# SinOncology/BreakID

Hardware: NVIDIA B200
Metric: read_pairs_per_sec_classified_clustered_refined (higher is better)
Workload: dtype u32/i64 integer + f64 (AHC distances)

## Files before the change

breakid_b200/csrc/bkid_api.cuh:

```cuda
#pragma once

#define GRID1(n, t) (unsigned)div_up((long long)(n), (t))

enum CounterSlot {
  CS_G = 0,
  CS_SD_OUT = 16,
  CS_SDF = 20,
  CS_SORT = 28,
  CS_TOTAL = 32,
  CS_HASH_ERR = 40,
  CS_MAXSPAN = 44,
  CS_FATAL = 46,
  CS_ROOTS = 48,
  CS_MISSING = 50,
  CS_DECODE = 52,
  CS_NC = 64,
  CS_XBAD = 65,
  CS_RG_TICKET = 66,
  CS_SORT_HEAP = 67
};

struct Scratch {
  DBuf keys, keys_alt, vals, vals_alt, hist, scan_tmp, a32, b32, c32, d32, e32;
  int ensure(long long n, cudaStream_t st)
  {
    size_t m = (size_t)std::max<long long>(n, 1);
    BK_TRY(keys.ensure(m * 8, 0, st)); BK_TRY(keys_alt.ensure(m * 8, 0, st));
    BK_TRY(vals.ensure(m * 4, 0, st)); BK_TRY(vals_alt.ensure(m * 4, 0, st));
    BK_TRY(hist.ensure(bk::radix_hist_elems(n) * 4, 0, st));
    BK_TRY(scan_tmp.ensure((bk::scan_tmp_elems(std::max<long long>((long long)bk::radix_hist_elems(n), n)) + 8) * 8, 0, st));
    BK_TRY(a32.ensure(m * 4 + 16, 0, st)); BK_TRY(b32.ensure(m * 4 + 16, 0, st)); BK_TRY(c32.ensure(m * 4 + 16, 0, st));
    BK_TRY(d32.ensure(m * 4 + 16, 0, st)); BK_TRY(e32.ensure(m * 4 + 16, 0, st));
    return 0;
  }
  bk::RadixTmp rt() { return bk::RadixTmp{keys_alt.as<uint64_t>(), vals_alt.as<uint32_t>(), hist.as<uint32_t>(), scan_tmp.as<unsigned long long>()}; }
  void release() { for (DBuf *b : {&keys, &keys_alt, &vals, &vals_alt, &hist, &scan_tmp, &a32, &b32, &c32, &d32, &e32}) b->release(); }
};

struct bkid_decoder;
static void decoder_free(bkid_ctx *c);

struct bkid_ctx {
  bkid_decoder *dec = nullptr;
  std::vector<int32_t> ex_iv;
  DBuf ex_tab, ex_lo, ex_len, ex_pre;
  long long n_excluded = 0;
  int device = 0, n_sm = 148;
  cudaStream_t st = nullptr, st2 = nullptr, st3 = nullptr;
  bkid_params prm;
  int nt = 0;
  std::vector<uint32_t> target_len;
  std::vector<std::string> names;
  std::string err;
  DBuf d_cum, d_bucket_rank, d_canon;
  long long n = 0, cap_n = 0;
  bool borrowed = false;
  DBuf flag, mapq, tid, pos, isize, endpos, cls, cand_bits;
  DBuf isize16, span16;
  int form_isize = 0, form_span = 0;
  long long reserve_hint = 0;
  const int16_t *p_isize16 = nullptr; const uint16_t *p_span16 = nullptr;
  long long n_x = 0;
  DBuf x_rec, x_mtid, x_mpos, x_nh;
  const uint16_t *p_flag = nullptr; const uint8_t *p_mapq = nullptr;
  const int32_t *p_tid = nullptr, *p_pos = nullptr, *p_isize = nullptr, *p_endpos = nullptr;
  const uint32_t *p_x_rec = nullptr; const int32_t *p_x_mtid = nullptr, *p_x_mpos = nullptr; const uint64_t *p_x_nh = nullptr;
  long long n_sa = 0, n_cig = 0, sa_bytes = 0, oc_bytes = 0;
  DBuf sa_rec, cig_off, cig_ops, sa_off, sa_txt, oc_off, oc_txt;
  DBuf seq_off, seq4, seq_len; long long seq_bytes = 0; bool have_seq = false;
  const uint32_t *p_seq_off = nullptr; const uint8_t *p_seq4 = nullptr; const int32_t *p_seq_len = nullptr;
  const uint32_t *p_sa_rec = nullptr, *p_cig_off = nullptr, *p_cig_ops = nullptr, *p_sa_off = nullptr, *p_oc_off = nullptr;
  const uint8_t *p_sa_txt = nullptr, *p_oc_txt = nullptr;
  std::vector<DBuf> nib;
  std::vector<uint64_t> nib_len;
  DBuf d_nib_ptr, d_nib_len;
  bool classified = false, have_stats = false, scanned = false, clustered = false, refined = false;
  double mean = 0, sd = 0;
  long long sum_abs = 0, cnt_insert = 0, sd_total = 0;
  unsigned long long sum_sq = 0, xmax = 0;
  long long n_cand_k1 = 0;
  int sd_kub = 0;
  bool sd_fast_pending = false;
  DBuf tile_cand, counters, cand_idx, cand, bucket_rank_of;
  long long n_cand = 0;
  DBuf pairs0, pairs_tmp, bucket_off0;
  long long np0 = 0; int nb = 0;
  DBuf X, Y, bucket_of_pair;
  DBuf cur1, curb1, seg1;
  long long n1 = 0;
  DBuf mem_pair, mem_bucket, mem_cluster;
  long long n2 = 0;
  std::vector<int32_t> roots_per_bucket;
  DBuf sdtab, sdlut; bool sd_prepared = false; double sd_mean = 0;
  DBuf clusters, clusters_out, sarows, work, cov, depth, evoff, valid, name_key, name_row;
  const void *rows_ptr = nullptr; long long n_rows = 0, n_evcap = 0; int maxspan = 1; bool clusters_ranked = false;
  long long n_clusters = 0, n_called = 0;
  Scratch sc;
  DBuf tmpA, tmpB, tmpC, tmpD, tmpE, tmpF, tmpG, tmpH;
  DBuf dist_send, dist_recv, dist_rows;
  DBuf sortheap;
  DBuf sortbig;
  DBuf dist_scalars;
  bkid_timings tm;
  cudaEvent_t ev[16];
  cudaEvent_t ev_run[2];
  cudaEvent_t ev_side[2];
  cudaEvent_t ev_w[4];
  bool k8_attr_set = false;
  bool sd_side_pending = false;
  bool maxspan_cached = false, maxspan_pending = false;
  long long launches0 = 0;
};

struct SubTimer {
  cudaStream_t st; bool on; std::vector<std::pair<std::string, cudaEvent_t>> ev;
  explicit SubTimer(cudaStream_t s) : st(s), on(getenv("BKID_DEBUG_TIMING") != nullptr) { mark("start"); }
  void mark(const char *name) { if (!on) return; cudaEvent_t e; cudaEventCreate(&e); cudaEventRecord(e, st); ev.push_back({name, e}); }
  ~SubTimer() {
    if (!on) return;
    cudaStreamSynchronize(st);
    for (size_t i = 1; i < ev.size(); ++i) { float ms = 0; cudaEventElapsedTime(&ms, ev[i - 1].second, ev[i].second); fprintf(stderr, "[bkid-timing] %-28s %8.3f ms\n", ev[i].first.c_str(), ms); }
    for (auto &e : ev) cudaEventDestroy(e.second);
  }
};

static int fail(bkid_ctx *c, int code, const std::string &msg)
{
  if (c) c->err = msg;
  else g_create_err = msg;
  return code;
}
#define CU(c, x) do { cudaError_t e__ = (x); if (e__ != cudaSuccess) { bk_set_cuda_error(e__, __FILE__, __LINE__); return fail((c), e__ == cudaErrorMemoryAllocation ? BKID_ERR_NOMEM : BKID_ERR_CUDA, g_last_cuda_err); } } while (0)
#define TRY(c, x) do { int rc__ = (x); if (rc__ != 0) { if ((c)->err.empty()) (c)->err = g_last_cuda_err; return rc__; } } while (0)

static int sync_check(bkid_ctx *c)
{
  CU(c, cudaStreamSynchronize(c->st));
  CU(c, cudaGetLastError());
  return 0;
}

static int exact_sort_segments(bkid_ctx *c, uint32_t *key, uint32_t *val, const uint32_t *seg_off, int nseg, long long n)
{
  if (n < 2 || nseg <= 0) return 0;
  cudaStream_t st = c->st;
  size_t seg_bytes = ((size_t)n / 2 + 16) * sizeof(Seg);
  TRY(c, c->tmpA.ensure(seg_bytes, 0, st));
  TRY(c, c->tmpB.ensure(seg_bytes, 0, st));
  TRY(c, c->tmpC.ensure(seg_bytes, 0, st));
  TRY(c, c->tmpD.ensure((size_t)n * 4 + 16, 0, st));
  TRY(c, c->tmpE.ensure((size_t)n * 4 + 16, 0, st));
  TRY(c, c->counters.ensure(256, 0, st));
  unsigned *cnt = c->counters.as<unsigned>() + CS_SORT;
  CU(c, cudaMemsetAsync(cnt, 0, 16, st));
  Seg *act[2] = {c->tmpA.as<Seg>(), c->tmpB.as<Seg>()};
  Seg *term = c->tmpC.as<Seg>();
  TRY(c, c->tmpH.ensure(seg_bytes, 0, st));
  Seg *small = c->tmpH.as<Seg>();
  TRY(c, c->sortheap.ensure(((size_t)n / IS_SMALL + 16) * sizeof(Seg), 0, st));
  Seg *heapl = c->sortheap.as<Seg>();
  unsigned *n_heap = c->counters.as<unsigned>() + CS_SORT_HEAP;
  CU(c, cudaMemsetAsync(n_heap, 0, 4, st));
  const bool big_possible = n > (long long)IS_BIG;
  const size_t maxbig = (size_t)(n / IS_BIG) + 2, maxtiles = (size_t)(n / IS_BTILE) + maxbig + 2;
  BigSeg *big[2] = {nullptr, nullptr};
  unsigned long long *bigcnt = nullptr, *status = nullptr;
  unsigned *tickets = nullptr;
  if (big_possible) {
    TRY(c, c->sortbig.ensure(64 + 2 * maxbig * sizeof(BigSeg) + maxtiles * 8, 0, st));
    char *base = (char *)c->sortbig.p;
    bigcnt = (unsigned long long *)base; tickets = (unsigned *)(base + 16);
    big[0] = (BigSeg *)(base + 64); big[1] = big[0] + maxbig;
    status = (unsigned long long *)(big[1] + maxbig);
    CU(c, cudaMemsetAsync(base, 0, 64, st));
    CU(c, cudaMemsetAsync(status, 0, maxtiles * 8, st));
  }
  BK_LAUNCH(is_init_roots, GRID1(nseg, 256), 256, 0, st, seg_off, nseg, act[0], cnt + 0, small, cnt + 3, term, cnt + 2, big[0], bigcnt);
  int lg = 0;
  for (long long t = n; t > 1; t >>= 1) ++lg;
  int max_levels = 2 * lg + 2;
  int cur = 0;
  bool any_big = big_possible;
  for (int level = 0; level < max_levels; ++level) {
    if (level > 0 && (level % 4) == 0) {
      unsigned h = 0;
      unsigned long long hb = 0;
      CU(c, cudaMemcpyAsync(&h, cnt + cur, 4, cudaMemcpyDeviceToHost, st));
      if (any_big) CU(c, cudaMemcpyAsync(&hb, bigcnt + cur, 8, cudaMemcpyDeviceToHost, st));
      CU(c, cudaStreamSynchronize(st));
      if (hb == 0) any_big = false;
      if (h == 0 && !any_big) break;
    }
    CU(c, cudaMemsetAsync(cnt + (cur ^ 1), 0, 4, st));
    if (any_big) {
      BK_LAUNCH(is_big_part, 592, IS_THREADS, 0, st, key, val, big[cur], bigcnt + cur, tickets, status, c->tmpD.as<uint32_t>(), c->tmpE.as<uint32_t>(),
                bigcnt + (cur ^ 1), tickets + 1, heapl, n_heap);
      BK_LAUNCH(is_big_swap, 592, IS_THREADS, 0, st, key, val, big[cur], bigcnt + cur, tickets + 1, c->tmpD.as<uint32_t>(), c->tmpE.as<uint32_t>(),
                act[cur ^ 1], cnt + (cur ^ 1), small, cnt + 3, term, cnt + 2, big[cur ^ 1], bigcnt + (cur ^ 1), tickets, status);
    }
    BK_LAUNCH(is_level, 592, IS_THREADS, 0, st, key, val, act[cur], cnt + cur, act[cur ^ 1], cnt + (cur ^ 1), small, cnt + 3, term, cnt + 2,
              c->tmpD.as<uint32_t>(), c->tmpE.as<uint32_t>(), heapl, n_heap);
    cur ^= 1;
  }
  BK_LAUNCH(is_heap, 148, 256, IS_HEAP_SMEM_ELEMS * 8 + 16, st, key, val, heapl, n_heap);
  BK_LAUNCH(is_small, 2368, ISS_WARPS * 32, 0, st, key, val, small, cnt + 3);
  BK_LAUNCH(is_terminal, 592, 128, 0, st, key, val, term, cnt + 2);
  return 0;
}

static int sort_current_by(bkid_ctx *c, uint32_t *cur, long long n, const uint32_t *coord, const uint32_t *seg_off, int nseg)
{
  if (n < 2) return 0;
  TRY(c, c->tmpF.ensure((size_t)n * 4 + 16, 0, c->st));
  uint32_t *key = c->tmpF.as<uint32_t>();
  BK_LAUNCH(gather_u32, GRID1(n, 256), 256, 0, c->st, coord, cur, n, key);
  return exact_sort_segments(c, key, cur, seg_off, nseg, n);
}

static int mask_pass(bkid_ctx *c, const uint32_t *cur, const uint32_t *curb, const uint32_t *seg, long long n, int nseg, const uint32_t *X, const uint32_t *Y,
                     long long distance, uint32_t *cur_out, uint32_t *curb_out, uint32_t *seg_out, long long *n_out)
{
  cudaStream_t st = c->st;
  if (n == 0) { CU(c, cudaMemsetAsync(seg_out, 0, (size_t)(nseg + 1) * 4, st)); *n_out = 0; return 0; }
  TRY(c, c->sc.ensure(n, st));
  uint32_t *cnt = c->sc.a32.as<uint32_t>(), *off = c->sc.b32.as<uint32_t>();
  unsigned long long *tot = (unsigned long long *)(c->counters.as<unsigned>() + CS_TOTAL);
  BK_LAUNCH(k4_mask_count, GRID1(n, 256), 256, 0, st, cur, curb, seg, n, X, Y, distance, cnt);
  bk::exclusive_scan<uint32_t, uint32_t>(cnt, off, n, c->sc.scan_tmp.as<unsigned long long>(), tot, st);
  unsigned long long h = 0;
  CU(c, cudaMemcpyAsync(&h, tot, 8, cudaMemcpyDeviceToHost, st));
  CU(c, cudaStreamSynchronize(st));
  BK_LAUNCH(k4_mask_write, GRID1(n, 256), 256, 0, st, cur, curb, n, cnt, off, cur_out, curb_out);
  BK_LAUNCH(k4_new_offsets, GRID1(nseg + 1, 256), 256, 0, st, seg, nseg, off, n, h, seg_out);
  *n_out = (long long)h;
  return 0;
// ... 200 lines not shown
    unsigned *rg_ticket = c->counters.as<unsigned>() + CS_RG_TICKET;
    CU(c, cudaMemsetAsync(rg_ticket, 0, 4, st));
    BK_LAUNCH(ahc_rg_ties, 148 * 4, 128, 0, st, v, g, curb, bucket_flag, RG_LO, bucket_events, head_pos, tot, rg_ticket);
    BK_LAUNCH(ahc_rg_write, GRID1(n, 256), 256, 0, st, v, g, curb, n, bucket_flag, RG_LO);
  }
  T_.mark("ahc: replay rank form (global)");
  BK_LAUNCH(ahc_bucket_exact, (unsigned)nseg, 32, 0, st, v, bucket_comp_off, (uint32_t)nseg, bucket_flag, 4096u);
  T_.mark("ahc: replay+exact");
  unsigned *cnt = c->counters.as<unsigned>() + CS_ROOTS;
  CU(c, cudaMemsetAsync(cnt, 0, 4, st));
  uint64_t *rkey = c->sc.keys.as<uint64_t>();
  uint32_t *rnode = c->sc.vals.as<uint32_t>();
  BK_LAUNCH(ahc_final_roots, GRID1(ncomp, 128), 128, 0, st, v, ncomp, rkey, rnode, cnt, merges_pb);
  unsigned nroot = 0;
  CU(c, cudaMemcpyAsync(&nroot, cnt, 4, cudaMemcpyDeviceToHost, st)); CU(c, cudaStreamSynchronize(st));
  std::vector<unsigned> merges(nseg);
  std::vector<uint32_t> segh(nseg + 1);
  CU(c, cudaMemcpyAsync(merges.data(), merges_pb, (size_t)nseg * 4, cudaMemcpyDeviceToHost, st));
  CU(c, cudaMemcpyAsync(segh.data(), seg, (size_t)(nseg + 1) * 4, cudaMemcpyDeviceToHost, st));
  CU(c, cudaStreamSynchronize(st));
  for (int b = 0; b < nseg; ++b) c->roots_per_bucket[b] = (int32_t)(segh[b + 1] - segh[b]) - (int32_t)merges[b];
  if (nroot == 0) return sync_check(c);
  bk::radix_sort_pairs(rkey, rnode, nroot, 0, 32 + bbits, c->sc.rt(), st);
  uint32_t *rsize = c->sc.a32.as<uint32_t>(), *roff = c->sc.b32.as<uint32_t>(), *rhead = c->sc.e32.as<uint32_t>();
  BK_LAUNCH(ahc_root_sizes, GRID1(nroot, 128), 128, 0, st, v, rkey, rnode, nroot, rsize, rhead);
  BK_LAUNCH(ahc_root_firsts, GRID1(nroot, 128), 128, 0, st, rhead, nroot, rkey, bucket_first_root);
  bk::exclusive_scan<uint32_t, uint32_t>(rsize, roff, nroot, stmp, tot, st);
  unsigned long long nm = 0;
  CU(c, cudaMemcpyAsync(&nm, tot, 8, cudaMemcpyDeviceToHost, st)); CU(c, cudaStreamSynchronize(st));
  size_t mb = (size_t)std::max<unsigned long long>(nm, 1) * 4 + 16;
  TRY(c, c->mem_pair.ensure(mb, 0, st)); TRY(c, c->mem_bucket.ensure(mb, 0, st)); TRY(c, c->mem_cluster.ensure(mb, 0, st));
  TRY(c, c->tmpE.ensure(mb, 0, st));
  BK_LAUNCH(ahc_emit, GRID1(nroot, 4), 128, 0, st, v, rkey, rnode, roff, bucket_first_root, nroot, c->tmpE.as<uint32_t>(), c->mem_cluster.as<int32_t>(), c->mem_bucket.as<uint32_t>());
  BK_LAUNCH(gather_u32, GRID1(nm, 256), 256, 0, st, cur, c->tmpE.as<uint32_t>(), (long long)nm, c->mem_pair.as<uint32_t>());
  c->n2 = (long long)nm;
  T_.mark("ahc: final roots+emit");
  return sync_check(c);
}

__global__ void fast_member_keys(const uint32_t *__restrict__ curb, const int32_t *__restrict__ cl, long long n, uint64_t *__restrict__ key, uint32_t *__restrict__ val)
{
  long long p = (long long)blockIdx.x * blockDim.x + threadIdx.x;
  if (p < n) { key[p] = ((uint64_t)curb[p] << 32) | (uint32_t)cl[p]; val[p] = (uint32_t)p; }
}
__global__ void fast_member_write(const uint64_t *__restrict__ key, const uint32_t *__restrict__ val, const uint32_t *__restrict__ cur, long long n,
                                  uint32_t *__restrict__ mem_pair, uint32_t *__restrict__ mem_bucket, int32_t *__restrict__ mem_cluster)
{
  long long p = (long long)blockIdx.x * blockDim.x + threadIdx.x;
  if (p < n) { mem_pair[p] = cur[val[p]]; mem_bucket[p] = (uint32_t)(key[p] >> 32); mem_cluster[p] = (int32_t)(key[p] & 0xffffffffu); }
}

static int cluster_fast(bkid_ctx *c, const uint32_t *cur, const uint32_t *curb, const uint32_t *seg, long long n, int nseg, const uint32_t *X, const uint32_t *Y, double w,
                        long long np0)
{
  cudaStream_t st = c->st;
  c->n2 = 0;
  c->roots_per_bucket.assign(nseg, 0);
  if (n == 0) return 0;
  int min_reads = c->prm.min_reads;
  TRY(c, c->sc.ensure(std::max(n, np0) + 8, st));
  size_t m = (size_t)n * 4 + 64, sb = (size_t)(nseg + 2) * 4;
  TRY(c, c->tmpG.ensure(4 * m + 4 * sb + (size_t)np0 * 8 + 64, 0, st));
  uint32_t *curA = c->tmpG.as<uint32_t>(), *curbA = curA + n + 8, *curB = curbA + n + 8, *curbB = curB + n + 8;
  uint32_t *segA = curbB + n + 8, *segB = segA + nseg + 2;
  uint32_t *k1 = segB + nseg + 2, *k2 = k1 + np0;
  uint32_t *keep = c->sc.a32.as<uint32_t>(), *off = c->sc.b32.as<uint32_t>();
  long long na = 0, nb2 = 0, nc = 0;
  BK_LAUNCH(fast_sweep, GRID1(nseg, 64), 64, 0, st, cur, seg, (uint32_t)nseg, X, w, min_reads, k1, keep);
  TRY(c, compact_pass(c, cur, curb, seg, n, nseg, keep, curA, curbA, segA, off, &na));
  TRY(c, sort_current_by(c, curA, na, Y, segA, nseg));
  if (na > 0) BK_LAUNCH(fast_sweep, GRID1(nseg, 64), 64, 0, st, curA, segA, (uint32_t)nseg, Y, w, min_reads, k2, keep);
  TRY(c, compact_pass(c, curA, curbA, segA, na, nseg, keep, curB, curbB, segB, off, &nb2));
  TRY(c, sort_current_by(c, curB, nb2, X, segB, nseg));
  if (nb2 == 0) return sync_check(c);
  int32_t *cl = (int32_t *)c->sc.c32.as<uint32_t>();
  int32_t *ncl = (int32_t *)c->sc.d32.as<uint32_t>();
  BK_LAUNCH(fast_number, GRID1(nseg, 64), 64, 0, st, curB, segB, (uint32_t)nseg, k1, k2, min_reads, cl, keep, ncl);
  CU(c, cudaMemcpyAsync(c->roots_per_bucket.data(), ncl, (size_t)nseg * 4, cudaMemcpyDeviceToHost, st));
  uint32_t *curC = curA, *curbC = curbA;
  bk::exclusive_scan<uint32_t, uint32_t>(keep, off, nb2, c->sc.scan_tmp.as<unsigned long long>(), (unsigned long long *)(c->counters.as<unsigned>() + CS_TOTAL), st);
  unsigned long long h = 0;
  CU(c, cudaMemcpyAsync(&h, c->counters.as<unsigned>() + CS_TOTAL, 8, cudaMemcpyDeviceToHost, st)); CU(c, cudaStreamSynchronize(st));
  nc = (long long)h;
  if (nc == 0) return 0;
  BK_LAUNCH(compact_write, GRID1(nb2, 256), 256, 0, st, curB, curbB, keep, off, nb2, curC, curbC);
  uint32_t *clC = c->sc.e32.as<uint32_t>();
  BK_LAUNCH(compact_write, GRID1(nb2, 256), 256, 0, st, (const uint32_t *)cl, curbB, keep, off, nb2, clC, c->sc.vals_alt.as<uint32_t>() );
  uint64_t *key = c->sc.keys.as<uint64_t>();
  uint32_t *val = c->sc.vals.as<uint32_t>();
  BK_LAUNCH(fast_member_keys, GRID1(nc, 256), 256, 0, st, curbC, (const int32_t *)clC, nc, key, val);
  int bbits = 1; while ((1ll << bbits) < nseg + 1) ++bbits;
  bk::radix_sort_pairs(key, val, nc, 0, 32 + bbits, c->sc.rt(), st);
  size_t mb = (size_t)nc * 4 + 16;
  TRY(c, c->mem_pair.ensure(mb, 0, st)); TRY(c, c->mem_bucket.ensure(mb, 0, st)); TRY(c, c->mem_cluster.ensure(mb, 0, st));
  BK_LAUNCH(fast_member_write, GRID1(nc, 256), 256, 0, st, key, val, curC, nc, c->mem_pair.as<uint32_t>(), c->mem_bucket.as<uint32_t>(), c->mem_cluster.as<int32_t>());
  c->n2 = nc;
  return sync_check(c);
}

extern "C" {

int bkid_abi_version(void) { return BKID_ABI_VERSION; }

const char *bkid_last_error(const bkid_ctx *ctx) { return ctx ? ctx->err.c_str() : g_create_err.c_str(); }

void bkid_default_params(bkid_params *p)
{
  p->qual = 20; p->times = 2; p->fast = 0; p->min_reads = 2; p->bp_pos_error = 2; p->mismatch_num = 10; p->sd_mult = 3; p->validate_align = 0;
}

bkid_ctx *bkid_create(int device, const bkid_header *hdr, const bkid_params *params)
{
  int ndev = 0;
  cudaError_t e = cudaGetDeviceCount(&ndev);
  if (e != cudaSuccess || ndev == 0) { g_create_err = std::string("no usable CUDA device (there is no CPU fallback): ") + cudaGetErrorString(e); return nullptr; }
  if (device < 0 || device >= ndev) { g_create_err = "device index out of range"; return nullptr; }
  if (!hdr || hdr->n_targets < 0) { g_create_err = "bad header"; return nullptr; }
  if (cudaSetDevice(device) != cudaSuccess) { g_create_err = "cudaSetDevice failed"; return nullptr; }
  bkid_ctx *c = new bkid_ctx();
  c->device = device;
  cudaDeviceGetAttribute(&c->n_sm, cudaDevAttrMultiProcessorCount, device);
  if (params) c->prm = *params; else bkid_default_params(&c->prm);
  if (cudaStreamCreateWithFlags(&c->st, cudaStreamNonBlocking) != cudaSuccess) { g_create_err = "cudaStreamCreate failed"; delete c; return nullptr; }
  cudaStreamCreateWithFlags(&c->st2, cudaStreamNonBlocking);
  cudaStreamCreateWithFlags(&c->st3, cudaStreamNonBlocking);
  for (auto &ev : c->ev) cudaEventCreate(&ev);
  for (auto &ev : c->ev_run) cudaEventCreate(&ev);
  for (auto &ev : c->ev_side) cudaEventCreate(&ev);
  for (auto &ev : c->ev_w) cudaEventCreateWithFlags(&ev, cudaEventDisableTiming);
  c->nt = hdr->n_targets;
  for (int i = 0; i < c->nt; ++i) { c->target_len.push_back(hdr->target_len[i]); c->names.emplace_back(hdr->target_name[i]); }
  int nt = c->nt, m = nt + 1;
  std::vector<uint32_t> cum(nt + 1, 0);
  for (int i = 0; i < nt; ++i) cum[i + 1] = cum[i] + c->target_len[i];
  std::vector<std::pair<std::string, int>> bn;
  for (int a = 0; a < m; ++a)
    for (int b = 0; b < m; ++b) bn.push_back({(a ? c->names[a - 1] : std::string("*")) + "_" + (b ? c->names[b - 1] : std::string("*")), a * m + b});
  std::sort(bn.begin(), bn.end());
  std::vector<int32_t> rank((size_t)m * m);
  for (size_t r = 0; r < bn.size(); ++r) rank[bn[r].second] = (int32_t)r;
  std::vector<uint64_t> canon(nt ? nt : 1);
  for (int i = 0; i < nt; ++i) canon[i] = chr_code((const uint8_t *)c->names[i].data(), (uint32_t)c->names[i].size());
  bool ok = c->d_cum.ensure((size_t)(nt + 1) * 4, 0, c->st) == 0 && c->d_bucket_rank.ensure(rank.size() * 4, 0, c->st) == 0 &&
            c->d_canon.ensure(canon.size() * 8, 0, c->st) == 0 && c->counters.ensure(1024, 0, c->st) == 0 &&
            c->d_nib_ptr.ensure((size_t)(nt + 1) * 8, 0, c->st) == 0 && c->d_nib_len.ensure((size_t)(nt + 1) * 8, 0, c->st) == 0;
  if (!ok) { g_create_err = "device allocation failed: " + g_last_cuda_err; delete c; return nullptr; }
  cudaMemcpy(c->d_cum.p, cum.data(), (size_t)(nt + 1) * 4, cudaMemcpyHostToDevice);
  cudaMemcpy(c->d_bucket_rank.p, rank.data(), rank.size() * 4, cudaMemcpyHostToDevice);
  cudaMemcpy(c->d_canon.p, canon.data(), canon.size() * 8, cudaMemcpyHostToDevice);
  cudaMemset(c->d_nib_ptr.p, 0, (size_t)(nt + 1) * 8);
  cudaMemset(c->d_nib_len.p, 0, (size_t)(nt + 1) * 8);
  c->nib.resize(nt); c->nib_len.assign(nt, 0);
  cudaFuncSetAttribute(sd_resolve, cudaFuncAttributeMaxDynamicSharedMemorySize, SD_BLOCK * 9);
  cudaFuncSetAttribute(is_heap, cudaFuncAttributeMaxDynamicSharedMemorySize, (int)(IS_HEAP_SMEM_ELEMS * 8 + 16));
  cudaFuncSetAttribute(ahc_replay_smem, cudaFuncAttributeMaxDynamicSharedMemorySize, 49 * 4096);
  cudaFuncSetAttribute(ahc_replay_rank, cudaFuncAttributeMaxDynamicSharedMemorySize, 49 * 4096);
  memset(&c->tm, 0, sizeof c->tm);
  if (cudaGetLastError() != cudaSuccess) { g_create_err = "CUDA error during create"; delete c; return nullptr; }
  return c;
}

void bkid_destroy(bkid_ctx *c)
{
  if (!c) return;
  cudaSetDevice(c->device);
  cudaStreamSynchronize(c->st);
  decoder_free(c);
  for (DBuf *b : {&c->d_cum, &c->d_bucket_rank, &c->d_canon, &c->flag, &c->mapq, &c->tid, &c->pos, &c->isize, &c->endpos, &c->isize16, &c->span16, &c->cand_bits, &c->x_rec, &c->x_mtid, &c->x_mpos, &c->x_nh, &c->cls,
                  &c->sa_rec, &c->cig_off, &c->cig_ops, &c->sa_off, &c->sa_txt, &c->oc_off, &c->oc_txt, &c->seq_off, &c->seq4, &c->seq_len, &c->d_nib_ptr, &c->d_nib_len, &c->tile_cand, &c->counters,
                  &c->cand_idx, &c->cand, &c->bucket_rank_of, &c->pairs0, &c->pairs_tmp, &c->bucket_off0, &c->X, &c->Y, &c->bucket_of_pair, &c->cur1, &c->curb1, &c->seg1, &c->mem_pair,
                  &c->mem_bucket, &c->mem_cluster, &c->sdtab, &c->sdlut, &c->clusters, &c->clusters_out, &c->sarows, &c->name_key, &c->name_row, &c->ex_tab, &c->ex_lo, &c->ex_len, &c->ex_pre, &c->work, &c->cov, &c->depth, &c->evoff, &c->valid, &c->tmpA, &c->tmpB, &c->tmpC, &c->tmpD, &c->tmpE, &c->tmpF, &c->tmpG, &c->tmpH, &c->dist_send, &c->dist_recv, &c->dist_rows, &c->dist_scalars, &c->sortbig, &c->sortheap})
    b->release();
  for (auto &b : c->nib) b.release();
  c->sc.release();
  for (auto &ev : c->ev) cudaEventDestroy(ev);
  for (auto &ev : c->ev_run) cudaEventDestroy(ev);
  for (auto &ev : c->ev_side) cudaEventDestroy(ev);
  for (auto &ev : c->ev_w) cudaEventDestroy(ev);
  cudaStreamDestroy(c->st2);
  cudaStreamDestroy(c->st3);
  cudaStreamDestroy(c->st);
  delete c;
}

static void invalidate(bkid_ctx *c)
{
  if (c->sd_side_pending || c->sd_fast_pending) { cudaStreamSynchronize(c->st2); c->sd_side_pending = false; c->sd_fast_pending = false; }
  if (c->maxspan_pending) { cudaStreamSynchronize(c->st3); c->maxspan_pending = false; }
  c->classified = c->have_stats = c->scanned = c->clustered = c->refined = false; c->sd_prepared = false; c->maxspan_cached = false;
}

static int reserve_impl(bkid_ctx *c, long long n, long long n_x, long long n_sa, long long n_cig, long long sa_b, long long oc_b)
{
  cudaStream_t st = c->st;
  if (c->borrowed) return fail(c, BKID_ERR_ARG, "context holds borrowed device columns; bkid_reset first");
  size_t k = (size_t)c->n;
  TRY(c, c->flag.ensure((size_t)n * 2 + 64, k * 2, st)); TRY(c, c->mapq.ensure((size_t)n + 64, k, st));
  TRY(c, c->tid.ensure((size_t)n * 4 + 64, k * 4, st)); TRY(c, c->pos.ensure((size_t)n * 4 + 64, k * 4, st));
  if (c->form_isize == 1) TRY(c, c->isize.ensure((size_t)n * 4 + 64, k * 4, st));
  if (c->form_isize == 2) TRY(c, c->isize16.ensure((size_t)n * 2 + 64, k * 2, st));
  if (c->form_span == 1) TRY(c, c->endpos.ensure((size_t)n * 4 + 64, k * 4, st));
  if (c->form_span == 2) TRY(c, c->span16.ensure((size_t)n * 2 + 64, k * 2, st));
  size_t kx = (size_t)c->n_x;
  TRY(c, c->x_rec.ensure((size_t)n_x * 4 + 64, kx * 4, st)); TRY(c, c->x_mtid.ensure((size_t)n_x * 4 + 64, kx * 4, st));
  TRY(c, c->x_mpos.ensure((size_t)n_x * 4 + 64, kx * 4, st)); TRY(c, c->x_nh.ensure((size_t)n_x * 16 + 64, kx * 16, st));
  size_t s = (size_t)c->n_sa;
  TRY(c, c->sa_rec.ensure((size_t)n_sa * 4 + 64, s * 4, st));
  TRY(c, c->cig_off.ensure((size_t)(n_sa + 1) * 4 + 64, (s + 1) * 4, st));
  TRY(c, c->sa_off.ensure((size_t)(n_sa + 1) * 4 + 64, (s + 1) * 4, st));
  TRY(c, c->oc_off.ensure((size_t)(n_sa + 1) * 4 + 64, (s + 1) * 4, st));
  TRY(c, c->cig_ops.ensure((size_t)n_cig * 4 + 64, (size_t)c->n_cig * 4, st));
  TRY(c, c->sa_txt.ensure((size_t)sa_b + 64, (size_t)c->sa_bytes, st));
  TRY(c, c->oc_txt.ensure((size_t)oc_b + 64, (size_t)c->oc_bytes, st));
  return 0;
}

int bkid_reserve(bkid_ctx *c, int64_t n, int64_t n_x, int64_t n_sa, int64_t n_cig, int64_t sa_b, int64_t oc_b)
{
  if (!c) return BKID_ERR_ARG;
  cudaSetDevice(c->device);
  c->reserve_hint = std::max<long long>(c->reserve_hint, n);
  return reserve_impl(c, std::max<long long>(n, c->n), std::max<long long>(n_x, c->n_x), std::max<long long>(n_sa, c->n_sa), std::max<long long>(n_cig, c->n_cig),
                      std::max<long long>(sa_b, c->sa_bytes), std::max<long long>(oc_b, c->oc_bytes));
}

__global__ void add_offset_u32(uint32_t *p, long long n, uint32_t d)
{
  long long i = (long long)blockIdx.x * blockDim.x + threadIdx.x;
  if (i < n) p[i] += d;
}

__global__ void widen_isize16(const int16_t *__restrict__ src, long long n, int32_t *__restrict__ dst)
{
  long long i = (long long)blockIdx.x * blockDim.x + threadIdx.x;
  if (i < n) dst[i] = (int32_t)src[i];
}
__global__ void widen_span16(const int32_t *__restrict__ pos, const uint16_t *__restrict__ span, long long n, int32_t *__restrict__ endpos)
{
  long long i = (long long)blockIdx.x * blockDim.x + threadIdx.x;
  if (i < n) endpos[i] = pos[i] + (int32_t)span[i];
}
__global__ void widen_tid_runs(const uint32_t *__restrict__ start, const int32_t *__restrict__ rtid, int nruns, long long n, int32_t *__restrict__ tid)
{
  long long i = (long long)blockIdx.x * blockDim.x + threadIdx.x;
  if (i >= n) return;
  int a = 0, b = nruns;
  while (b - a > 1) { int m = (a + b) >> 1; if ((long long)start[m] <= i) a = m; else b = m; }
  tid[i] = rtid[a];
}

static void set_ptrs(bkid_ctx *c)
{
  c->p_flag = c->flag.as<uint16_t>(); c->p_mapq = c->mapq.as<uint8_t>(); c->p_tid = c->tid.as<int32_t>(); c->p_pos = c->pos.as<int32_t>();
  c->p_isize = c->form_isize == 2 ? nullptr : c->isize.as<int32_t>(); c->p_isize16 = c->form_isize == 2 ? c->isize16.as<int16_t>() : nullptr;
  c->p_endpos = c->form_span == 2 ? nullptr : c->endpos.as<int32_t>(); c->p_span16 = c->form_span == 2 ? c->span16.as<uint16_t>() : nullptr;
  c->p_x_rec = c->x_rec.as<uint32_t>(); c->p_x_mtid = c->x_mtid.as<int32_t>(); c->p_x_mpos = c->x_mpos.as<int32_t>(); c->p_x_nh = c->x_nh.as<uint64_t>();
  c->p_sa_rec = c->sa_rec.as<uint32_t>(); c->p_cig_off = c->cig_off.as<uint32_t>(); c->p_cig_ops = c->cig_ops.as<uint32_t>();
  c->p_seq_off = c->seq_off.as<uint32_t>(); c->p_seq4 = c->seq4.as<uint8_t>(); c->p_seq_len = c->seq_len.as<int32_t>();
  c->p_sa_off = c->sa_off.as<uint32_t>(); c->p_sa_txt = c->sa_txt.as<uint8_t>(); c->p_oc_off = c->oc_off.as<uint32_t>(); c->p_oc_txt = c->oc_txt.as<uint8_t>();
}

static int settle_forms(bkid_ctx *c, int want_isize, int want_span, long long n_new)
{
  cudaStream_t st = c->st;
  long long n0 = c->n;
  size_t cap = (size_t)std::max<long long>(n0 + n_new, c->reserve_hint);
  if (c->form_isize == 0) c->form_isize = want_isize;
  else if (c->form_isize == 2 && want_isize == 1) {
    TRY(c, c->isize.ensure(cap * 4 + 64, 0, st));
    if (n0) BK_LAUNCH(widen_isize16, GRID1(n0, 256), 256, 0, st, c->isize16.as<int16_t>(), n0, c->isize.as<int32_t>());
    c->form_isize = 1;
  }
  if (c->form_span == 0) c->form_span = want_span;
  else if (c->form_span == 2 && want_span == 1) {
    TRY(c, c->endpos.ensure(cap * 4 + 64, 0, st));
    if (n0) BK_LAUNCH(widen_span16, GRID1(n0, 256), 256, 0, st, c->pos.as<int32_t>(), c->span16.as<uint16_t>(), n0, c->endpos.as<int32_t>());
    c->form_span = 1;
  }
  return 0;
}

static int push_impl(bkid_ctx *c, const bkid_batch *b, cudaMemcpyKind kind)
{
  if (!c || !b || b->n < 0 || b->n_sa < 0 || b->n_x < 0) return c ? fail(c, BKID_ERR_ARG, "bad batch") : BKID_ERR_ARG;
  if (b->n > 0 && ((!b->isize && !b->isize16) || (!b->endpos && !b->span16) || (!b->tid && (b->n_tid_runs <= 0 || !b->tid_run_start || !b->tid_run_tid))))
    return fail(c, BKID_ERR_ARG, "bad batch: a dense column is missing in both its wide and its narrow form");
  cudaSetDevice(c->device);
  cudaStream_t st = c->st;
  if ((unsigned long long)(c->n + b->n) >= 0xffffffffull) return fail(c, BKID_ERR_ARG, "more than 2^32-1 records per context");
  invalidate(c);
  cudaEventRecord(c->ev[0], st);
  long long n0 = c->n, s0 = c->n_sa, x0 = c->n_x;
  uint32_t ncig = 0, nsa_b = 0, noc_b = 0;
  if (b->n_sa > 0) {
    if (kind == cudaMemcpyHostToDevice) { ncig = b->cig_off[b->n_sa]; nsa_b = b->sa_off[b->n_sa]; noc_b = b->oc_off[b->n_sa]; }
    else {
      CU(c, cudaMemcpy(&ncig, b->cig_off + b->n_sa, 4, cudaMemcpyDeviceToHost));
      CU(c, cudaMemcpy(&nsa_b, b->sa_off + b->n_sa, 4, cudaMemcpyDeviceToHost));
      CU(c, cudaMemcpy(&noc_b, b->oc_off + b->n_sa, 4, cudaMemcpyDeviceToHost));
    }
  }
  if (b->n > 0) TRY(c, settle_forms(c, b->isize ? 1 : 2, b->endpos ? 1 : 2, b->n));
  TRY(c, reserve_impl(c, std::max<long long>(n0 + b->n, c->reserve_hint), x0 + b->n_x, s0 + b->n_sa, c->n_cig + ncig, c->sa_bytes + nsa_b, c->oc_bytes + noc_b));
  size_t n = (size_t)b->n;
  if (n) {
    cudaStream_t sw = c->st3;
    const bool widen_i = b->isize16 && !b->isize && c->form_isize == 1, widen_s = b->span16 && !b->endpos && c->form_span == 1;
    size_t stage = (widen_i ? n * 2 : 0) + (widen_s ? n * 2 : 0) + (b->tid ? 0 : (size_t)b->n_tid_runs * 8) + 64;
    TRY(c, c->tmpH.ensure(stage, 0, st));
    char *sp = (char *)c->tmpH.p;
    bool widened = false;
    if (b->tid) CU(c, cudaMemcpyAsync(c->tid.as<int32_t>() + n0, b->tid, n * 4, kind, st));
    else {
      uint32_t *rs = (uint32_t *)sp; sp += (size_t)b->n_tid_runs * 4;
      int32_t *rt = (int32_t *)sp; sp += (size_t)b->n_tid_runs * 4;
      CU(c, cudaMemcpyAsync(rs, b->tid_run_start, (size_t)b->n_tid_runs * 4, kind, st));
      CU(c, cudaMemcpyAsync(rt, b->tid_run_tid, (size_t)b->n_tid_runs * 4, kind, st));
      CU(c, cudaEventRecord(c->ev_w[0], st)); CU(c, cudaStreamWaitEvent(sw, c->ev_w[0], 0));
      BK_LAUNCH(widen_tid_runs, GRID1(n, 256), 256, 0, sw, rs, rt, (int)b->n_tid_runs, (long long)n, c->tid.as<int32_t>() + n0);
      widened = true;
    }
    if (c->form_isize == 2) CU(c, cudaMemcpyAsync(c->isize16.as<int16_t>() + n0, b->isize16, n * 2, kind, st));
    else if (b->isize) CU(c, cudaMemcpyAsync(c->isize.as<int32_t>() + n0, b->isize, n * 4, kind, st));
    else {
      int16_t *s16 = (int16_t *)sp; sp += n * 2;
      CU(c, cudaMemcpyAsync(s16, b->isize16, n * 2, kind, st));
      CU(c, cudaEventRecord(c->ev_w[1], st)); CU(c, cudaStreamWaitEvent(sw, c->ev_w[1], 0));
      BK_LAUNCH(widen_isize16, GRID1(n, 256), 256, 0, sw, s16, (long long)n, c->isize.as<int32_t>() + n0);
      widened = true;
    }
    CU(c, cudaMemcpyAsync(c->pos.as<int32_t>() + n0, b->pos, n * 4, kind, st));
    if (c->form_span == 2) CU(c, cudaMemcpyAsync(c->span16.as<uint16_t>() + n0, b->span16, n * 2, kind, st));
    else if (b->endpos) CU(c, cudaMemcpyAsync(c->endpos.as<int32_t>() + n0, b->endpos, n * 4, kind, st));
    else {
      uint16_t *e16 = (uint16_t *)sp; sp += n * 2;
      CU(c, cudaMemcpyAsync(e16, b->span16, n * 2, kind, st));
      CU(c, cudaEventRecord(c->ev_w[2], st)); CU(c, cudaStreamWaitEvent(sw, c->ev_w[2], 0));
      BK_LAUNCH(widen_span16, GRID1(n, 256), 256, 0, sw, c->pos.as<int32_t>() + n0, e16, (long long)n, c->endpos.as<int32_t>() + n0);
      widened = true;
    }
    CU(c, cudaMemcpyAsync(c->flag.as<uint16_t>() + n0, b->flag, n * 2, kind, st));
    CU(c, cudaMemcpyAsync(c->mapq.as<uint8_t>() + n0, b->mapq, n, kind, st));
    if (widened) { CU(c, cudaEventRecord(c->ev_w[3], sw)); CU(c, cudaStreamWaitEvent(st, c->ev_w[3], 0)); }
  }
  size_t nx = (size_t)b->n_x;
  if (nx) {
    CU(c, cudaMemcpyAsync(c->x_rec.as<uint32_t>() + x0, b->x_rec, nx * 4, kind, st));
    CU(c, cudaMemcpyAsync(c->x_mtid.as<int32_t>() + x0, b->x_mtid, nx * 4, kind, st));
    CU(c, cudaMemcpyAsync(c->x_mpos.as<int32_t>() + x0, b->x_mpos, nx * 4, kind, st));
    CU(c, cudaMemcpyAsync(c->x_nh.as<uint64_t>() + 2 * x0, b->x_name_hash, nx * 16, kind, st));
    if (n0) BK_LAUNCH(add_offset_u32, GRID1(nx, 256), 256, 0, st, c->x_rec.as<uint32_t>() + x0, (long long)nx, (uint32_t)n0);
  }
  size_t ns = (size_t)b->n_sa;
  if (ns) {
    CU(c, cudaMemcpyAsync(c->sa_rec.as<uint32_t>() + s0, b->sa_rec, ns * 4, kind, st));
    CU(c, cudaMemcpyAsync(c->cig_off.as<uint32_t>() + s0, b->cig_off, (ns + 1) * 4, kind, st));
    CU(c, cudaMemcpyAsync(c->sa_off.as<uint32_t>() + s0, b->sa_off, (ns + 1) * 4, kind, st));
    CU(c, cudaMemcpyAsync(c->oc_off.as<uint32_t>() + s0, b->oc_off, (ns + 1) * 4, kind, st));
    if (ncig) CU(c, cudaMemcpyAsync(c->cig_ops.as<uint32_t>() + c->n_cig, b->cig_ops, (size_t)ncig * 4, kind, st));
    if (nsa_b) CU(c, cudaMemcpyAsync(c->sa_txt.as<uint8_t>() + c->sa_bytes, b->sa_txt, nsa_b, kind, st));
    if (noc_b) CU(c, cudaMemcpyAsync(c->oc_txt.as<uint8_t>() + c->oc_bytes, b->oc_txt, noc_b, kind, st));
    if (n0) BK_LAUNCH(add_offset_u32, GRID1(ns, 256), 256, 0, st, c->sa_rec.as<uint32_t>() + s0, (long long)ns, (uint32_t)n0);
    if (c->n_cig) BK_LAUNCH(add_offset_u32, GRID1(ns + 1, 256), 256, 0, st, c->cig_off.as<uint32_t>() + s0, (long long)ns + 1, (uint32_t)c->n_cig);
    if (c->sa_bytes) BK_LAUNCH(add_offset_u32, GRID1(ns + 1, 256), 256, 0, st, c->sa_off.as<uint32_t>() + s0, (long long)ns + 1, (uint32_t)c->sa_bytes);
    if (c->oc_bytes) BK_LAUNCH(add_offset_u32, GRID1(ns + 1, 256), 256, 0, st, c->oc_off.as<uint32_t>() + s0, (long long)ns + 1, (uint32_t)c->oc_bytes);
  } else if (s0 == 0) {
    CU(c, cudaMemsetAsync(c->cig_off.p, 0, 4, st)); CU(c, cudaMemsetAsync(c->sa_off.p, 0, 4, st)); CU(c, cudaMemsetAsync(c->oc_off.p, 0, 4, st));
  }
  if (ns) {
    if (b->seq_off && b->seq4 && b->seq_len && (s0 == 0 || c->have_seq)) {
      uint32_t nseq_b = 0;
      if (kind == cudaMemcpyHostToDevice) nseq_b = b->seq_off[ns];
      else CU(c, cudaMemcpy(&nseq_b, b->seq_off + ns, 4, cudaMemcpyDeviceToHost));
      TRY(c, c->seq_off.ensure((size_t)(s0 + ns + 1) * 4 + 64, (size_t)(s0 + 1) * 4, st));
      TRY(c, c->seq_len.ensure((size_t)(s0 + ns) * 4 + 64, (size_t)s0 * 4, st));
      TRY(c, c->seq4.ensure((size_t)c->seq_bytes + nseq_b + 64, (size_t)c->seq_bytes, st));
      CU(c, cudaMemcpyAsync(c->seq_off.as<uint32_t>() + s0, b->seq_off, (ns + 1) * 4, kind, st));
      CU(c, cudaMemcpyAsync(c->seq_len.as<int32_t>() + s0, b->seq_len, ns * 4, kind, st));
      if (nseq_b) CU(c, cudaMemcpyAsync(c->seq4.as<uint8_t>() + c->seq_bytes, b->seq4, nseq_b, kind, st));
      if (c->seq_bytes) BK_LAUNCH(add_offset_u32, GRID1(ns + 1, 256), 256, 0, st, c->seq_off.as<uint32_t>() + s0, (long long)ns + 1, (uint32_t)c->seq_bytes);
      c->seq_bytes += nseq_b; c->have_seq = true;
    } else c->have_seq = false;
  }
  c->n += b->n; c->n_x += b->n_x; c->n_sa += b->n_sa; c->n_cig += ncig; c->sa_bytes += nsa_b; c->oc_bytes += noc_b;
  set_ptrs(c);
  cudaEventRecord(c->ev[1], st);
  TRY(c, sync_check(c));
  float ms = 0; cudaEventElapsedTime(&ms, c->ev[0], c->ev[1]);
  c->tm.h2d += ms;
  return 0;
}

int bkid_push_batch(bkid_ctx *c, const bkid_batch *b) { return push_impl(c, b, cudaMemcpyHostToDevice); }

int bkid_push_batch_device(bkid_ctx *c, const bkid_batch *b)
{
  if (!c || !b) return BKID_ERR_ARG;
  if (c->n == 0 && !c->borrowed && c->flag.p == nullptr) {
    cudaSetDevice(c->device);
    if ((unsigned long long)b->n >= 0xffffffffull) return fail(c, BKID_ERR_ARG, "more than 2^32-1 records per context");
    if (b->n > 0 && (!b->tid || (!b->isize && !b->isize16) || (!b->endpos && !b->span16)))
      return fail(c, BKID_ERR_ARG, "bkid_push_batch_device needs tid and the insert-size / span columns (wide or narrow) resident on the device");
    invalidate(c);
    c->borrowed = true;
    c->n = b->n; c->n_sa = b->n_sa; c->n_x = b->n_x;
    c->p_flag = b->flag; c->p_mapq = b->mapq; c->p_tid = b->tid; c->p_pos = b->pos;
    c->p_isize = b->isize; c->p_isize16 = b->isize ? nullptr : b->isize16;
    c->p_endpos = b->endpos; c->p_span16 = b->endpos ? nullptr : b->span16;
    c->form_isize = b->isize ? 1 : 2; c->form_span = b->endpos ? 1 : 2;
    c->p_x_rec = b->x_rec; c->p_x_mtid = b->x_mtid; c->p_x_mpos = b->x_mpos; c->p_x_nh = b->x_name_hash;
    c->p_sa_rec = b->sa_rec; c->p_cig_off = b->cig_off; c->p_cig_ops = b->cig_ops; c->p_sa_off = b->sa_off; c->p_sa_txt = b->sa_txt;
    c->p_oc_off = b->oc_off; c->p_oc_txt = b->oc_txt;
    c->p_seq_off = b->seq_off; c->p_seq4 = b->seq4; c->p_seq_len = b->seq_len; c->have_seq = b->seq_off && b->seq4 && b->seq_len;
    return 0;
  }
  return push_impl(c, b, cudaMemcpyDeviceToDevice);
}

int bkid_reset(bkid_ctx *c)
{
  if (!c) return BKID_ERR_ARG;
  cudaSetDevice(c->device);
  cudaStreamSynchronize(c->st);
  invalidate(c);
  c->n = c->n_x = c->n_sa = c->n_cig = c->sa_bytes = c->oc_bytes = 0;
  c->seq_bytes = 0; c->have_seq = false;
  c->borrowed = false;
  c->form_isize = c->form_span = 0;
  set_ptrs(c);
  memset(&c->tm, 0, sizeof c->tm);
  c->launches0 = g_bk_launches;
  return 0;
}

int bkid_set_exclude(bkid_ctx *c, int64_t n_iv, const int32_t *tid, const int32_t *beg, const int32_t *end)
{
  if (!c || n_iv < 0 || (n_iv > 0 && (!tid || !beg || !end))) return c ? fail(c, BKID_ERR_ARG, "bad exclude intervals") : BKID_ERR_ARG;
  cudaSetDevice(c->device);
  std::vector<std::array<int32_t, 3>> v;
  for (int64_t k = 0; k < n_iv; ++k) {
    if (tid[k] < 0 || tid[k] >= c->nt) return fail(c, BKID_ERR_ARG, "exclude interval on an unknown target");
    int32_t b = beg[k] < 0 ? 0 : beg[k];
    if (end[k] > b) v.push_back({tid[k], b, end[k]});
  }
  std::sort(v.begin(), v.end());
  c->ex_iv.clear();
  for (auto &x : v) {
    size_t m = c->ex_iv.size();
    if (m && c->ex_iv[m - 3] == x[0] && x[1] <= c->ex_iv[m - 1]) { if (x[2] > c->ex_iv[m - 1]) c->ex_iv[m - 1] = x[2]; }
    else { c->ex_iv.push_back(x[0]); c->ex_iv.push_back(x[1]); c->ex_iv.push_back(x[2]); }
  }
  invalidate(c);
  return 0;
}

static ISizeCol isize_col(const bkid_ctx *c) { return ISizeCol{c->p_isize, c->p_isize16}; }

static int classify_impl(bkid_ctx *c)
{
  if (c->classified) return 0;
  cudaStream_t st = c->st;
  long long n = c->n;
  int ntiles = div_up(std::max<long long>(n, 1), K1_TILE);
  TRY(c, c->cls.ensure((size_t)n + 64, 0, st));
  TRY(c, c->cand_bits.ensure((size_t)n / 8 + 64, 0, st));
  unsigned long long *g = (unsigned long long *)(c->counters.as<unsigned>() + CS_G);
  CU(c, cudaMemsetAsync(g, 0, 64, st));
  cudaEventRecord(c->ev[2], st);
  const bool i16 = c->p_isize16 != nullptr, s16 = c->p_span16 != nullptr;
  if (n > 0) {
    uint8_t *cls = c->cls.as<uint8_t>();
    int occ = 0;
    if (i16 && s16) cudaOccupancyMaxActiveBlocksPerMultiprocessor(&occ, k1_classify<true, true>, K1_THREADS, 0);
    else if (i16) cudaOccupancyMaxActiveBlocksPerMultiprocessor(&occ, k1_classify<true, false>, K1_THREADS, 0);
    else if (s16) cudaOccupancyMaxActiveBlocksPerMultiprocessor(&occ, k1_classify<false, true>, K1_THREADS, 0);
    else cudaOccupancyMaxActiveBlocksPerMultiprocessor(&occ, k1_classify<false, false>, K1_THREADS, 0);
    ntiles = std::min(ntiles, c->n_sm * std::max(occ, 1));
    if (i16 && s16) BK_LAUNCH((k1_classify<true, true>), (unsigned)ntiles, K1_THREADS, 0, st, c->p_flag, c->p_mapq, c->p_isize, c->p_isize16, c->p_span16, n, c->prm.qual, cls, c->cand_bits.as<uint8_t>(), g);
    else if (i16) BK_LAUNCH((k1_classify<true, false>), (unsigned)ntiles, K1_THREADS, 0, st, c->p_flag, c->p_mapq, c->p_isize, c->p_isize16, c->p_span16, n, c->prm.qual, cls, c->cand_bits.as<uint8_t>(), g);
    else if (s16) BK_LAUNCH((k1_classify<false, true>), (unsigned)ntiles, K1_THREADS, 0, st, c->p_flag, c->p_mapq, c->p_isize, c->p_isize16, c->p_span16, n, c->prm.qual, cls, c->cand_bits.as<uint8_t>(), g);
    else BK_LAUNCH((k1_classify<false, false>), (unsigned)ntiles, K1_THREADS, 0, st, c->p_flag, c->p_mapq, c->p_isize, c->p_isize16, c->p_span16, n, c->prm.qual, cls, c->cand_bits.as<uint8_t>(), g);
  }
  cudaEventRecord(c->ev[3], st);
  int n_iv = (int)(c->ex_iv.size() / 3);
  c->n_excluded = 0;
  unsigned long long ne = 0;
  if (n_iv > 0 && n > 0) {
    TRY(c, c->ex_tab.ensure((size_t)n_iv * 12 + 64, 0, st)); TRY(c, c->ex_lo.ensure((size_t)n_iv * 4 + 64, 0, st));
    TRY(c, c->ex_len.ensure((size_t)n_iv * 4 + 64, 0, st)); TRY(c, c->ex_pre.ensure((size_t)(n_iv + 1) * 8 + 64, 0, st));
    CU(c, cudaMemcpyAsync(c->ex_tab.p, c->ex_iv.data(), (size_t)n_iv * 12, cudaMemcpyHostToDevice, st));
    BK_LAUNCH(ex_ranges, GRID1(n_iv, 128), 128, 0, st, c->p_tid, c->p_pos, n, c->ex_tab.as<int32_t>(), n_iv, c->ex_lo.as<uint32_t>(), c->ex_len.as<uint32_t>());
    BK_LAUNCH(ex_prefix, 1, 32, 0, st, c->ex_len.as<uint32_t>(), n_iv, c->ex_pre.as<unsigned long long>());
    BK_LAUNCH(ex_apply, 148 * 8, 256, 0, st, c->ex_lo.as<uint32_t>(), c->ex_pre.as<unsigned long long>(), n_iv, isize_col(c), c->cls.as<uint8_t>(), c->cand_bits.as<uint8_t>(), g);
    CU(c, cudaMemcpyAsync(&ne, c->ex_pre.as<unsigned long long>() + n_iv, 8, cudaMemcpyDeviceToHost, st));
  }
  unsigned long long h[6] = {0, 0, 0, 0, 0, 0};
  CU(c, cudaMemcpyAsync(h, g, 48, cudaMemcpyDeviceToHost, st));
  TRY(c, sync_check(c));
  c->n_excluded = (long long)ne;
  float ms = 0; cudaEventElapsedTime(&ms, c->ev[2], c->ev[3]);
  c->tm.classify = ms;
  c->sum_abs = (long long)h[G_SUM]; c->cnt_insert = (long long)h[G_CNT]; c->sum_sq = h[G_SQ]; c->n_cand_k1 = (long long)h[G_CAND]; c->xmax = h[G_XMAX];
  if (s16) { c->maxspan = (int)h[G_SPAN] + 1; c->maxspan_cached = true; }
  c->classified = true;
  c->tm.n_records = n;
  return 0;
}

static int sd_upper_binade(unsigned long long sum_abs, unsigned long long cnt, unsigned long long sum_sq, unsigned long long xmax)
{
  if (cnt == 0) return 0;
  if (xmax > 65535ull) return 51;
  unsigned __int128 V = (unsigned __int128)sum_sq * cnt - (unsigned __int128)sum_abs * sum_abs;
  unsigned __int128 T = V / cnt + 1;
  T += (T >> 30) + 2 * (unsigned __int128)cnt + 1024;
  if (T >> 51) return 51;
  int k = 0;
  while ((T >> (k + 1)) != 0) ++k;
  return k;
}

static int sd_prepare_impl(bkid_ctx *c, double mean, cudaStream_t st = nullptr)
{
  if (!st) st = c->st;
  long long n = c->n;
  c->sd_prepared = false;
  if (n <= 0 || c->cnt_insert <= 0) return 0;
  int nb = div_up(std::max<long long>(n, 1), SD_BLOCK);
  TRY(c, c->sdtab.ensure((size_t)nb * (8 + SD_K * 4 + 4 + 8) + 256, 0, st));
  TRY(c, c->sdlut.ensure((size_t)SD_LUT * 8, 0, st));
  char *bp = (char *)c->sdtab.p;
  long long *blkF = (long long *)bp; bp += (size_t)nb * 8;
  double *blkA = (double *)bp; bp += (size_t)nb * 8;
  uint32_t *blkCum = (uint32_t *)bp; bp += (size_t)nb * SD_K * 4;
  uint32_t *blkN = (uint32_t *)bp;
  BK_LAUNCH(sd_build_lut, SD_LUT / 256, 256, 0, st, mean, c->sdlut.as<unsigned long long>());
  BK_LAUNCH(sd_block_stats, (unsigned)nb, SD_THREADS, 0, st, c->cls.as<uint8_t>(), isize_col(c), n, mean, c->sdlut.as<unsigned long long>(), blkF, blkCum, blkN, blkA);
  c->sd_prepared = true; c->sd_mean = mean;
  return 0;
}

static int sd_partial_impl(bkid_ctx *c, double mean, long long t_in, long long *t_out)
{
  cudaStream_t st = c->st;
  long long n = c->n;
  *t_out = t_in;
  if (n <= 0 || c->cnt_insert <= 0) return 0;
  SubTimer T_(st);
  if (!c->sd_prepared || c->sd_mean != mean) TRY(c, sd_prepare_impl(c, mean));
  T_.mark("sd: block stats");
  int nb = div_up(std::max<long long>(n, 1), SD_BLOCK);
  char *bp = (char *)c->sdtab.p;
  long long *blkF = (long long *)bp; bp += (size_t)nb * 8;
  double *blkA = (double *)bp; bp += (size_t)nb * 8;
  uint32_t *blkCum = (uint32_t *)bp; bp += (size_t)nb * SD_K * 4;
  uint32_t *blkN = (uint32_t *)bp;
  long long *out = (long long *)(c->counters.as<unsigned>() + CS_SD_OUT);
  BK_LAUNCH(sd_resolve, 1, SDR_T, SD_BLOCK * 9, st, c->cls.as<uint8_t>(), isize_col(c), n, mean, nb, blkF, blkCum, blkN, blkA, t_in, out);
  T_.mark("sd: resolve");
  long long h[2] = {0, 0};
  CU(c, cudaMemcpyAsync(h, out, 16, cudaMemcpyDeviceToHost, st));
  TRY(c, sync_check(c));
  if (h[1]) {
    BK_LAUNCH(sd_sequential, 1, 1, 0, st, c->cls.as<uint8_t>(), isize_col(c), n, mean, t_in, out);
    CU(c, cudaMemcpyAsync(h, out, 16, cudaMemcpyDeviceToHost, st));
    TRY(c, sync_check(c));
  }
  *t_out = h[0];
  return 0;
}

static int sd_fast_launch(bkid_ctx *c, double mean, int kub, cudaStream_t st)
{
  long long n = c->n;
  unsigned long long *out = (unsigned long long *)(c->counters.as<unsigned>() + CS_SDF);
  CU(c, cudaMemsetAsync(out, 0, 24, st));
  c->sd_kub = kub;
  if (n <= 0 || c->cnt_insert <= 0) return 0;
  double thr = 1.0 - ldexp(1.0, kub - 53);
  int occ = 0;
  if (c->p_isize16) cudaOccupancyMaxActiveBlocksPerMultiprocessor(&occ, sd_fast<true>, 256, 0);
  else cudaOccupancyMaxActiveBlocksPerMultiprocessor(&occ, sd_fast<false>, 256, 0);
  const int grid = c->n_sm * std::max(occ, 1);
  if (c->p_isize16) BK_LAUNCH((sd_fast<true>), grid, 256, 0, st, c->cls.as<uint8_t>(), c->p_isize, c->p_isize16, n, mean, thr, out);
  else BK_LAUNCH((sd_fast<false>), grid, 256, 0, st, c->cls.as<uint8_t>(), c->p_isize, c->p_isize16, n, mean, thr, out);
  return 0;
}
static int sd_fast_collect(bkid_ctx *c, cudaStream_t st, unsigned long long *F, unsigned long long *E)
{
  unsigned long long h[3] = {0, 0, 0};
  CU(c, cudaMemcpyAsync(h, c->counters.as<unsigned>() + CS_SDF, 24, cudaMemcpyDeviceToHost, st));
  CU(c, cudaStreamSynchronize(st));
  CU(c, cudaGetLastError());
  *F = h[0]; *E = h[2] ? ~0ull : h[1];
  if (c->sd_kub >= 51 && c->cnt_insert > 0) *E = ~0ull;
  return 0;
}

static int side_launch(bkid_ctx *c)
{
  cudaStream_t s2 = c->st2;
  long long n = c->n;
  c->mean = (double)c->sum_abs / (double)c->cnt_insert;
  cudaEventRecord(c->ev_side[0], s2);
  TRY(c, sd_fast_launch(c, c->mean, sd_upper_binade((unsigned long long)c->sum_abs, (unsigned long long)c->cnt_insert, c->sum_sq, c->xmax), s2));
  cudaEventRecord(c->ev_side[1], s2);
  c->sd_fast_pending = true;
  if (!c->maxspan_cached) {
    int *mx = (int *)(c->counters.as<unsigned>() + CS_MAXSPAN);
    CU(c, cudaMemsetAsync(mx, 0, 4, c->st3));
    if (n > 0) BK_LAUNCH(max_span_kernel, 1184, 256, 0, c->st3, c->p_pos, c->p_endpos, n, mx);
    c->maxspan_pending = true;
  }
  return 0;
}

static int side_collect(bkid_ctx *c)
{
  unsigned long long F = 0, E = 0;
  TRY(c, sd_fast_collect(c, c->st2, &F, &E));
  c->sd_fast_pending = false;
  float ms = 0; cudaEventElapsedTime(&ms, c->ev_side[0], c->ev_side[1]);
  long long total = (long long)F;
  if (E != 0 && c->n > 0 && c->cnt_insert > 0) {
    cudaEventRecord(c->ev[4], c->st);
    TRY(c, sd_partial_impl(c, c->mean, 0, &total));
    cudaEventRecord(c->ev[5], c->st);
    TRY(c, sync_check(c));
    float ms2 = 0; cudaEventElapsedTime(&ms2, c->ev[4], c->ev[5]);
    ms += ms2;
  }
  c->tm.insert_stats = ms;
  c->sd_total = total;
  c->sd = sqrt((double)c->sd_total / (double)c->cnt_insert);
  c->have_stats = true;
  return 0;
}

static int maxspan_collect(bkid_ctx *c)
{
  if (!c->maxspan_pending) return 0;
  int maxspan = 0;
  CU(c, cudaMemcpyAsync(&maxspan, c->counters.as<unsigned>() + CS_MAXSPAN, 4, cudaMemcpyDeviceToHost, c->st3));
  CU(c, cudaStreamSynchronize(c->st3));
  CU(c, cudaGetLastError());
  c->maxspan = maxspan + 1; c->maxspan_cached = true; c->maxspan_pending = false;
  return 0;
}

int bkid_insert_stats(bkid_ctx *c, double *mean, double *sd)
{
  if (!c) return BKID_ERR_ARG;
  cudaSetDevice(c->device);
  c->err.clear();
  TRY(c, classify_impl(c));
  if (!c->have_stats) {
    cudaStream_t st = c->st;
    c->mean = (double)c->sum_abs / (double)c->cnt_insert;
    cudaEventRecord(c->ev[4], st);
    unsigned long long F = 0, E = 0;
    const bool general_only = getenv("BKID_SD_GENERAL") != nullptr;
    if (!general_only) {
      TRY(c, sd_fast_launch(c, c->mean, sd_upper_binade((unsigned long long)c->sum_abs, (unsigned long long)c->cnt_insert, c->sum_sq, c->xmax), st));
      TRY(c, sd_fast_collect(c, st, &F, &E));
    }
    long long t = (long long)F;
    if ((general_only || E != 0) && c->n > 0 && c->cnt_insert > 0) TRY(c, sd_partial_impl(c, c->mean, 0, &t));
    cudaEventRecord(c->ev[5], st);
    TRY(c, sync_check(c));
    float ms = 0; cudaEventElapsedTime(&ms, c->ev[4], c->ev[5]);
    c->tm.insert_stats = ms;
    c->sd_total = t;
    c->sd = sqrt((double)c->sd_total / (double)c->cnt_insert);
    c->have_stats = true;
  }
  if (mean) *mean = c->mean;
  if (sd) *sd = c->sd;
  return 0;
}

static int extract_candidates(bkid_ctx *c, unsigned long long index_offset, bool with_keys)
{
  TRY(c, classify_impl(c));
  cudaStream_t st = c->st;
  long long n = c->n, nx = c->n_x;
  long long cap = std::min<long long>(c->n_cand_k1, nx);
  c->n_cand = cap;
  unsigned *cs = c->counters.as<unsigned>();
  CU(c, cudaMemsetAsync(cs + CS_NC, 0, 8, st));
  TRY(c, c->cand.ensure((size_t)(cap + 1) * sizeof(bkid_cand), 0, st));
  if (nx <= 0 || n <= 0) return 0;
  int ntiles = div_up(nx, KX_TILE);
  TRY(c, c->sc.ensure(std::max<long long>(cap, ntiles) + 8, st));
  TRY(c, c->tile_cand.ensure((size_t)(ntiles + 1) * 4 * 2 + (size_t)ntiles * KX_THREADS + 64, 0, st));
  uint32_t *tile_cnt = c->tile_cand.as<uint32_t>(), *tile_off = tile_cnt + ntiles + 1;
  uint8_t *is_cand = (uint8_t *)(tile_off + ntiles + 1);
  unsigned long long *tot = (unsigned long long *)(cs + CS_TOTAL);
  BK_LAUNCH(kx_count, (unsigned)ntiles, KX_THREADS, 0, st, c->p_x_rec, nx, c->cand_bits.as<uint8_t>(), n, tile_cnt, is_cand, (int *)(cs + CS_XBAD));
  bk::exclusive_scan<uint32_t, uint32_t>(tile_cnt, tile_off, ntiles, c->sc.scan_tmp.as<unsigned long long>(), tot, st);
  CU(c, cudaMemcpyAsync(cs + CS_NC, tot, 4, cudaMemcpyDeviceToDevice, st));
  if (cap > 0)
    BK_LAUNCH(kx_write, (unsigned)ntiles, KX_THREADS, 0, st, c->p_x_rec, nx, is_cand, n, tile_off, c->p_flag, c->p_mapq, c->p_tid, c->p_pos, c->p_x_mtid, c->p_x_mpos, c->p_x_nh,
              index_offset, c->cand.as<bkid_cand>(), with_keys ? c->sc.keys.as<uint64_t>() : (uint64_t *)nullptr, c->sc.vals.as<uint32_t>());
  return 0;
}
static int check_candidates(bkid_ctx *c, const unsigned *h_nc_bad)
{
  if (h_nc_bad[1]) return fail(c, BKID_ERR_ARG, "the sparse mate/name table is not strictly ascending or points outside the batch (x_rec)");
  if ((long long)h_nc_bad[0] != c->n_cand_k1)
    return fail(c, BKID_ERR_ARG, "a discordant-scan candidate is missing from the sparse mate/name table (x_rec must list every record that is not a proper pair)");
  return 0;
}

static int join_presort(bkid_ctx *c, const bkid_cand *cand, long long nc, const uint32_t *nc_dev, bool keys_ready)
{
  cudaStream_t st = c->st;
  if (nc <= 0) return 0;
  TRY(c, c->sc.ensure(nc + 8, st));
  uint64_t *key = c->sc.keys.as<uint64_t>();
  uint32_t *val = c->sc.vals.as<uint32_t>();
  if (!keys_ready) BK_LAUNCH(k2_cand_keys, GRID1(nc, 256), 256, 0, st, cand, nc, key, val);
  if (bk::radix_sort_pairs(key, val, nc, 0, 32, c->sc.rt(), st, nc_dev) < 0) return fail(c, BKID_ERR_ARG, "more than 2^30 candidates");
  size_t maxp = (size_t)nc / 2 + 1;
  TRY(c, c->pairs_tmp.ensure(maxp * sizeof(bkid_pair), 0, st));
  return 0;
}

static int join_emit(bkid_ctx *c, const bkid_cand *cand, long long nc, const uint32_t *nc_dev, double w, bool check_table, long long *np_out)
{
  cudaStream_t st = c->st;
  *np_out = 0;
  unsigned *cs = c->counters.as<unsigned>();
  unsigned long long *tot = (unsigned long long *)(cs + CS_TOTAL);
  uint64_t *key = c->sc.keys.as<uint64_t>();
  uint32_t *val = c->sc.vals.as<uint32_t>();
  uint32_t *flag = c->sc.a32.as<uint32_t>(), *off = c->sc.b32.as<uint32_t>(), *mate = c->sc.c32.as<uint32_t>();
  int *big = (int *)(cs + CS_HASH_ERR);
  unsigned long long np = 0; int hbig = 0; unsigned hnc[2] = {0, 0};
  for (int attempt = 0; attempt < 2 && nc > 0; ++attempt) {
    CU(c, cudaMemsetAsync(big, 0, 4, st));
    CU(c, cudaMemsetAsync(mate, 0xff, (size_t)nc * 4, st));
    if (attempt == 1 && bk::radix_sort_pairs(key, val, nc, 32, 64, c->sc.rt(), st, nc_dev) < 0) return fail(c, BKID_ERR_ARG, "more than 2^30 candidates");
    BK_LAUNCH(k2_join, GRID1(nc, 256), 256, 0, st, key, val, nc_dev, (uint32_t)nc, cand, attempt == 0 ? 32 : 64, attempt == 0 ? 64u : 4096u, w, mate, big);
    BK_LAUNCH(k2_mate_flags, GRID1(nc, 256), 256, 0, st, mate, nc, flag);
    bk::exclusive_scan<uint32_t, uint32_t>(flag, off, nc, c->sc.scan_tmp.as<unsigned long long>(), tot, st);
    BK_LAUNCH(k2_build_pairs, GRID1(nc, 256), 256, 0, st, mate, off, nc, cand, c->d_cum.as<uint32_t>(), c->nt, c->d_bucket_rank.as<int32_t>(), c->pairs_tmp.as<bkid_pair>());
    CU(c, cudaMemcpyAsync(&np, tot, 8, cudaMemcpyDeviceToHost, st));
    CU(c, cudaMemcpyAsync(&hbig, big, 4, cudaMemcpyDeviceToHost, st));
    CU(c, cudaMemcpyAsync(hnc, cs + CS_NC, 8, cudaMemcpyDeviceToHost, st));
    TRY(c, sync_check(c));
    if (!hbig) break;
    if (attempt == 1) return fail(c, BKID_ERR_HASH, "more than 4096 records share a 64-bit read-name hash without sharing the name");
  }
  if (check_table) { if (nc <= 0) { CU(c, cudaMemcpyAsync(hnc, cs + CS_NC, 8, cudaMemcpyDeviceToHost, st)); TRY(c, sync_check(c)); } TRY(c, check_candidates(c, hnc)); }
  *np_out = (long long)np;
  return 0;
}

static int join_candidates(bkid_ctx *c, const bkid_cand *cand, long long nc, double w, long long *np_out)
{
  TRY(c, join_presort(c, cand, nc, nullptr, false));
  return join_emit(c, cand, nc, nullptr, w, false, np_out);
}

static int set_pairs(bkid_ctx *c, const bkid_pair *pairs, long long np, bool ordered)
{
  cudaStream_t st = c->st;
  c->np0 = np; c->nb = 0;
  if (np <= 0) return 0;
  unsigned long long *tot = (unsigned long long *)(c->counters.as<unsigned>() + CS_TOTAL);
  TRY(c, c->sc.ensure(np + 8, st));
  TRY(c, c->pairs0.ensure((size_t)np * sizeof(bkid_pair), 0, st));
  unsigned long long *pkey = (unsigned long long *)c->sc.keys.as<uint64_t>();
  uint32_t *pslot = c->sc.vals.as<uint32_t>();
  BK_LAUNCH(k2_pair_keys, GRID1(np, 256), 256, 0, st, pairs, np, ordered ? 1 : 0, pkey, pslot);
  int rbits = 1; while ((1ll << rbits) < (long long)(c->nt + 1) * (c->nt + 1) + 1) ++rbits;
  if (bk::radix_sort_pairs((uint64_t *)pkey, pslot, np, ordered ? PAIR_IDX_BITS : 0, PAIR_IDX_BITS + rbits, c->sc.rt(), st) < 0) return fail(c, BKID_ERR_ARG, "more than 2^30 pairs");
  uint32_t *bh = c->sc.a32.as<uint32_t>(), *bhx = c->sc.b32.as<uint32_t>();
  BK_LAUNCH(k2_gather_pairs, GRID1(np, 256), 256, 0, st, pairs, pslot, pkey, np, c->pairs0.as<bkid_pair>(), bh);
  bk::exclusive_scan<uint32_t, uint32_t>(bh, bhx, np, c->sc.scan_tmp.as<unsigned long long>(), tot, st);
  unsigned long long nbk = 0;
  CU(c, cudaMemcpyAsync(&nbk, tot, 8, cudaMemcpyDeviceToHost, st));
  TRY(c, sync_check(c));
  c->nb = (int)nbk;
  TRY(c, c->bucket_off0.ensure((size_t)(nbk + 2) * 4, 0, st));
  TRY(c, c->bucket_rank_of.ensure((size_t)(nbk + 2) * 4, 0, st));
  BK_LAUNCH(k2_bucket_ids, GRID1(np, 256), 256, 0, st, c->pairs0.as<bkid_pair>(), bh, bhx, np, c->bucket_off0.as<uint32_t>(), c->bucket_rank_of.as<int32_t>());
  uint32_t npu = (uint32_t)np;
  CU(c, cudaMemcpyAsync(c->bucket_off0.as<uint32_t>() + nbk, &npu, 4, cudaMemcpyHostToDevice, st));
  TRY(c, c->X.ensure((size_t)np * 4 + 64, 0, st)); TRY(c, c->Y.ensure((size_t)np * 4 + 64, 0, st)); TRY(c, c->bucket_of_pair.ensure((size_t)np * 4 + 64, 0, st));
  BK_LAUNCH(pair_xy, GRID1(np, 256), 256, 0, st, c->pairs0.as<bkid_pair>(), np, c->X.as<uint32_t>(), c->Y.as<uint32_t>(), c->bucket_of_pair.as<uint32_t>());
  return sync_check(c);
}

int bkid_scan(bkid_ctx *c, double w, int64_t *n_pairs)
{
  if (!c) return BKID_ERR_ARG;
  cudaSetDevice(c->device);
  c->err.clear();
  cudaStream_t st = c->st;
  TRY(c, classify_impl(c));
  cudaEventRecord(c->ev[6], st);
  TRY(c, extract_candidates(c, 0ull, true));
  long long np = 0;
  const uint32_t *nc_dev = c->counters.as<unsigned>() + CS_NC;
  TRY(c, join_presort(c, c->cand.as<bkid_cand>(), c->n_cand, nc_dev, true));
  TRY(c, join_emit(c, c->cand.as<bkid_cand>(), c->n_cand, nc_dev, w, true, &np));
  cudaEventRecord(c->ev[7], st);
  TRY(c, set_pairs(c, c->pairs_tmp.as<bkid_pair>(), np, true));
  cudaEventRecord(c->ev[8], st);
  TRY(c, sync_check(c));
  float ms = 0;
  cudaEventElapsedTime(&ms, c->ev[6], c->ev[7]); c->tm.join = ms;
  cudaEventElapsedTime(&ms, c->ev[7], c->ev[8]); c->tm.bucket_sort = ms;
  c->tm.n_candidates = c->n_cand; c->tm.n_pairs = c->np0;
  c->scanned = true; c->clustered = c->refined = false;
  if (n_pairs) *n_pairs = c->np0;
// ... 132 lines not shown
  return v;
}

static int refine_coverage(bkid_ctx *c, double dist)
{
  cudaStream_t st = c->st;
  uint32_t ncl = (uint32_t)c->n_clusters;
  TRY(c, classify_impl(c));
  TRY(c, c->sc.ensure((long long)ncl + 8, st));
  TRY(c, c->work.ensure((size_t)(ncl + 1) * sizeof(ClusterWork), 0, st));
  TRY(c, c->cov.ensure((size_t)(2 * ncl + 2) * 4, 0, st));
  TRY(c, c->depth.ensure((size_t)(2 * ncl + 2) * 4, 0, st));
  TRY(c, c->evoff.ensure((size_t)(ncl + 2) * 4, 0, st));
  if (ncl == 0) return 0;
  RefineView v = refine_view(c);
  int w = (int)dist;
  unsigned long long *tot = (unsigned long long *)(c->counters.as<unsigned>() + CS_TOTAL);
  uint32_t *evcap = c->sc.a32.as<uint32_t>();
  BK_LAUNCH(k7_regions, GRID1(ncl, 128), 128, 0, st, v, c->clusters.as<bkid_cluster_rec>(), ncl, w, c->work.as<ClusterWork>(), evcap);
  bk::exclusive_scan<uint32_t, uint32_t>(evcap, c->evoff.as<uint32_t>(), ncl, c->sc.scan_tmp.as<unsigned long long>(), tot, st);
  BK_LAUNCH(k7_coverage, GRID1(ncl, 4), 128, 0, st, v, c->work.as<ClusterWork>(), ncl, c->cov.as<uint32_t>());
  unsigned long long nev = 0;
  CU(c, cudaMemcpyAsync(&nev, tot, 8, cudaMemcpyDeviceToHost, st));
  TRY(c, sync_check(c));
  c->n_evcap = (long long)nev;
  return 0;
}

static int refine_vote(bkid_ctx *c)
{
  cudaStream_t st = c->st;
  uint32_t ncl = (uint32_t)c->n_clusters;
  if (ncl == 0) return 0;
  TRY(c, c->sc.ensure(std::max<long long>(ncl, c->n_rows) + 8, st));
  TRY(c, c->name_key.ensure((size_t)(c->n_rows + 1) * 8, 0, st));
  TRY(c, c->name_row.ensure((size_t)(c->n_rows + 1) * 4, 0, st));
  if (c->n_rows > 0) {
    BK_LAUNCH(k7_name_keys, GRID1(c->n_rows, 256), 256, 0, st, (const EvRow *)c->rows_ptr, c->n_rows, c->name_key.as<uint64_t>(), c->name_row.as<uint32_t>());
    bk::radix_sort_pairs(c->name_key.as<uint64_t>(), c->name_row.as<uint32_t>(), c->n_rows, 0, 32, c->sc.rt(), st);
  }
  RefineView v = refine_view(c);
  unsigned long long *tot = (unsigned long long *)(c->counters.as<unsigned>() + CS_TOTAL);
  ClusterWork *work = c->work.as<ClusterWork>();
  uint32_t *entcnt = c->sc.c32.as<uint32_t>(), *entoff = c->sc.d32.as<uint32_t>();
  TRY(c, c->valid.ensure((size_t)(ncl + 2) * 4, 0, st));
  TRY(c, c->tmpC.ensure((size_t)(c->n_evcap + 1) * 4, 0, st));
  int *fatal = (int *)(c->counters.as<unsigned>() + CS_FATAL);
  CU(c, cudaMemsetAsync(fatal, 0, 4, st));
  BK_LAUNCH((k7_collect<false>), ncl, RF_THREADS, 0, st, v, c->clusters.as<bkid_cluster_rec>(), ncl, work, c->cov.as<uint32_t>(), c->evoff.as<uint32_t>(),
            c->tmpC.as<uint32_t>(), (const uint32_t *)nullptr, (int2 *)nullptr);
  BK_LAUNCH(k7_entry_counts, GRID1(ncl, 128), 128, 0, st, work, ncl, entcnt, fatal);
  bk::exclusive_scan<uint32_t, uint32_t>(entcnt, entoff, ncl, c->sc.scan_tmp.as<unsigned long long>(), tot, st);
  unsigned long long nent = 0; int hf = 0;
  CU(c, cudaMemcpyAsync(&nent, tot, 8, cudaMemcpyDeviceToHost, st));
  CU(c, cudaMemcpyAsync(&hf, fatal, 4, cudaMemcpyDeviceToHost, st));
  TRY(c, sync_check(c));
  if (hf) return fail(c, BKID_ERR_CIGAR, "error cigar: a complementary split alignment has no clip (reference exits at src/BreakID.cc:954-968)");
  TRY(c, c->tmpD.ensure((size_t)(nent + 1) * sizeof(int2), 0, st));
  BK_LAUNCH((k7_collect<true>), ncl, RF_THREADS, 0, st, v, c->clusters.as<bkid_cluster_rec>(), ncl, work, c->cov.as<uint32_t>(), c->evoff.as<uint32_t>(),
            c->tmpC.as<uint32_t>(), entoff, c->tmpD.as<int2>());
  BK_LAUNCH(k8_vote, ncl, RF_THREADS, 0, st, c->clusters.as<bkid_cluster_rec>(), ncl, work, entoff, c->tmpD.as<int2>(), c->prm.bp_pos_error, c->valid.as<uint32_t>());
  if (nent > K8_SMALL) {
    TRY(c, c->tmpE.ensure((size_t)(nent + 1) * 8, 0, st));
    TRY(c, c->tmpF.ensure((size_t)(nent + 1) * 4, 0, st));
    if (!c->k8_attr_set) { cudaFuncSetAttribute(k8_vote_big, cudaFuncAttributeMaxDynamicSharedMemorySize, (int)(K8_BIG_SMEM_KEYS * 8)); c->k8_attr_set = true; }
    BK_LAUNCH(k8_vote_big, ncl, K8_BIG_THREADS, K8_BIG_SMEM_KEYS * 8, st, c->clusters.as<bkid_cluster_rec>(), ncl, work, entoff, c->tmpD.as<int2>(), c->tmpE.as<uint64_t>(),
              c->tmpF.as<uint32_t>(), c->prm.bp_pos_error, c->valid.as<uint32_t>());
  }
  c->tm.n_evidence = (long long)nent;
  return 0;
}

static int refine_depth(bkid_ctx *c)
{
  uint32_t ncl = (uint32_t)c->n_clusters;
  if (ncl == 0) return 0;
  RefineView v = refine_view(c);
  BK_LAUNCH(k9_depth, GRID1(ncl, 4), 128, 0, c->st, v, c->clusters.as<bkid_cluster_rec>(), c->valid.as<uint32_t>(), ncl, c->depth.as<uint32_t>());
  return 0;
}

static int refine_finish(bkid_ctx *c)
{
  cudaStream_t st = c->st;
  uint32_t ncl = (uint32_t)c->n_clusters;
  c->n_called = 0;
  if (ncl == 0) return 0;
  RefineView v = refine_view(c);
  unsigned long long *tot = (unsigned long long *)(c->counters.as<unsigned>() + CS_TOTAL);
  BK_LAUNCH(k10_finish, GRID1(ncl, 128), 128, 0, st, v, c->clusters.as<bkid_cluster_rec>(), c->valid.as<uint32_t>(), c->depth.as<uint32_t>(), ncl);
  uint32_t *voff = c->sc.b32.as<uint32_t>();
  bk::exclusive_scan<uint32_t, uint32_t>(c->valid.as<uint32_t>(), voff, ncl, c->sc.scan_tmp.as<unsigned long long>(), tot, st);
  unsigned long long nv = 0;
  CU(c, cudaMemcpyAsync(&nv, tot, 8, cudaMemcpyDeviceToHost, st));
  TRY(c, sync_check(c));
  TRY(c, c->clusters_out.ensure((size_t)(ncl + 1) * sizeof(bkid_cluster_rec), 0, st));
  BK_LAUNCH(compact_clusters, GRID1(ncl, 128), 128, 0, st, c->clusters.as<bkid_cluster_rec>(), c->valid.as<uint32_t>(), voff, ncl, c->clusters_out.as<bkid_cluster_rec>());
  c->n_called = (long long)nv;
  return sync_check(c);
}

int bkid_refine(bkid_ctx *c, double dist, int64_t *n_called)
{
  if (!c) return BKID_ERR_ARG;
  if (!c->clustered) return fail(c, BKID_ERR_ARG, "bkid_refine before bkid_cluster");
  cudaSetDevice(c->device);
  c->err.clear();
  cudaStream_t st = c->st;
  c->n_called = 0;
  cudaEventRecord(c->ev[13], st);
  if (c->n_clusters > 0) {
    TRY(c, refine_build_rows(c));
    TRY(c, maxspan_collect(c));
    if (!c->maxspan_cached) TRY(c, refine_local_maxspan(c, &c->maxspan));
    cudaEventRecord(c->ev[14], st);
    TRY(c, refine_coverage(c, dist));
    TRY(c, refine_vote(c));
    TRY(c, refine_depth(c));
    TRY(c, refine_finish(c));
  } else cudaEventRecord(c->ev[14], st);
  cudaEventRecord(c->ev[15], st);
  TRY(c, sync_check(c));
  float ms = 0;
  cudaEventElapsedTime(&ms, c->ev[13], c->ev[14]); c->tm.evidence = ms;
  cudaEventElapsedTime(&ms, c->ev[14], c->ev[15]); c->tm.refine = ms;
  c->tm.n_sa = c->n_sa; c->tm.n_called = c->n_called;
  c->refined = true;
  if (n_called) *n_called = c->n_called;
  return 0;
}


int bkid_shard_insert_partial(bkid_ctx *c, int64_t *sum_abs, int64_t *count, uint64_t *sum_sq, uint64_t *max_abs)
{
  if (!c) return BKID_ERR_ARG;
  cudaSetDevice(c->device); c->err.clear();
  TRY(c, classify_impl(c));
  *sum_abs = c->sum_abs; *count = c->cnt_insert;
  if (sum_sq) *sum_sq = c->sum_sq;
  if (max_abs) *max_abs = c->xmax;
  return 0;
}

int bkid_sd_upper_binade(uint64_t sum_abs, uint64_t count, uint64_t sum_sq, uint64_t max_abs)
{
  return sd_upper_binade(sum_abs, count, sum_sq, max_abs);
}

int bkid_shard_sd_fast(bkid_ctx *c, double mean, int32_t upper_binade)
{
  if (!c) return BKID_ERR_ARG;
  cudaSetDevice(c->device); c->err.clear();
  TRY(c, classify_impl(c));
  TRY(c, sd_fast_launch(c, mean, upper_binade, c->st2));
  c->sd_fast_pending = true;
  return 0;
}

int bkid_shard_sd_fast_collect(bkid_ctx *c, uint64_t *sum_floor, uint64_t *n_correctable)
{
  if (!c || !sum_floor || !n_correctable) return BKID_ERR_ARG;
  cudaSetDevice(c->device); c->err.clear();
  unsigned long long F = 0, E = 0;
  TRY(c, sd_fast_collect(c, c->st2, &F, &E));
  c->sd_fast_pending = false;
  *sum_floor = F; *n_correctable = E == ~0ull ? (uint64_t)1 << 62 : E;
  return 0;
}

int bkid_shard_sd_prepare(bkid_ctx *c, double mean)
{
  if (!c) return BKID_ERR_ARG;
  cudaSetDevice(c->device); c->err.clear();
  TRY(c, classify_impl(c));
  TRY(c, sd_prepare_impl(c, mean, c->st2));
  CU(c, cudaEventRecord(c->ev_side[1], c->st2));
  c->sd_side_pending = true;
  return 0;
}

int bkid_shard_sd_partial(bkid_ctx *c, double mean, int64_t t_in, int64_t *t_out)
{
  if (!c) return BKID_ERR_ARG;
  cudaSetDevice(c->device); c->err.clear();
  TRY(c, classify_impl(c));
  if (c->sd_side_pending) { CU(c, cudaStreamWaitEvent(c->st, c->ev_side[1], 0)); c->sd_side_pending = false; }
  long long t = 0;
  TRY(c, sd_partial_impl(c, mean, (long long)t_in, &t));
  *t_out = t;
  return 0;
}

int bkid_shard_set_stats(bkid_ctx *c, double mean, double sd)
{
  if (!c) return BKID_ERR_ARG;
  c->mean = mean; c->sd = sd; c->have_stats = true;
  return 0;
}

int bkid_shard_candidates(bkid_ctx *c, uint64_t index_offset, const bkid_cand **dev, int64_t *n)
{
  if (!c) return BKID_ERR_ARG;
  cudaSetDevice(c->device); c->err.clear();
  TRY(c, extract_candidates(c, index_offset, false));
  unsigned hnc[2] = {0, 0};
  CU(c, cudaMemcpyAsync(hnc, c->counters.as<unsigned>() + CS_NC, 8, cudaMemcpyDeviceToHost, c->st));
  TRY(c, sync_check(c));
  TRY(c, check_candidates(c, hnc));
  *dev = c->cand.as<bkid_cand>(); *n = c->n_cand;
  return 0;
}

int bkid_shard_join(bkid_ctx *c, const bkid_cand *dev_cand, int64_t n, double w, const bkid_pair **dev_pairs, int64_t *n_pairs)
{
  if (!c) return BKID_ERR_ARG;
  cudaSetDevice(c->device); c->err.clear();
  long long np = 0;
  TRY(c, join_candidates(c, dev_cand, n, w, &np));
  *dev_pairs = c->pairs_tmp.as<bkid_pair>(); *n_pairs = np;
  return 0;
}

int bkid_shard_set_pairs(bkid_ctx *c, const bkid_pair *dev_pairs, int64_t n)
{
  if (!c) return BKID_ERR_ARG;
  cudaSetDevice(c->device); c->err.clear();
  TRY(c, set_pairs(c, dev_pairs, n, false));
  c->tm.n_pairs = c->np0;
  c->scanned = true; c->clustered = c->refined = false;
  return 0;
}

__global__ void cluster_bucket_to_rank(bkid_cluster_rec *cl, uint32_t n, const int32_t *__restrict__ rank_of)
{
  uint32_t i = blockIdx.x * blockDim.x + threadIdx.x;
  if (i < n) cl[i].bucket = rank_of[cl[i].bucket];
}

int bkid_shard_clusters(bkid_ctx *c, const bkid_cluster_rec **dev, int64_t *n)
{
  if (!c || !c->clustered) return c ? fail(c, BKID_ERR_ARG, "bkid_shard_clusters before bkid_cluster") : BKID_ERR_ARG;
  cudaSetDevice(c->device); c->err.clear();
  if (c->n_clusters > 0 && !c->clusters_ranked) {
    BK_LAUNCH(cluster_bucket_to_rank, GRID1(c->n_clusters, 128), 128, 0, c->st, c->clusters.as<bkid_cluster_rec>(), (uint32_t)c->n_clusters, c->bucket_rank_of.as<int32_t>());
    c->clusters_ranked = true;
  }
  TRY(c, sync_check(c));
  *dev = c->clusters.as<bkid_cluster_rec>(); *n = c->n_clusters;
  return 0;
}

int bkid_shard_set_clusters(bkid_ctx *c, const bkid_cluster_rec *dev, int64_t n)
{
  if (!c || n < 0) return BKID_ERR_ARG;
  cudaSetDevice(c->device); c->err.clear();
  TRY(c, c->clusters.ensure((size_t)(n + 1) * sizeof(bkid_cluster_rec), 0, c->st));
  if (n > 0 && dev != c->clusters.as<bkid_cluster_rec>()) CU(c, cudaMemcpyAsync(c->clusters.p, dev, (size_t)n * sizeof(bkid_cluster_rec), cudaMemcpyDeviceToDevice, c->st));
  c->n_clusters = n; c->clusters_ranked = true; c->clustered = true; c->refined = false;
  return sync_check(c);
}

int bkid_shard_sa_rows(bkid_ctx *c, const bkid_sarow **dev, int64_t *n)
{
  if (!c) return BKID_ERR_ARG;
  cudaSetDevice(c->device); c->err.clear();
  TRY(c, refine_build_rows(c));
  TRY(c, sync_check(c));
  *dev = (const bkid_sarow *)c->sarows.p; *n = c->n_sa;
  return 0;
}

int bkid_shard_set_sa_rows(bkid_ctx *c, const bkid_sarow *dev, int64_t n)
{
  if (!c || n < 0) return BKID_ERR_ARG;
  c->rows_ptr = dev; c->n_rows = n;
  return 0;
}

int bkid_shard_maxspan(bkid_ctx *c, int32_t *maxspan)
{
  if (!c) return BKID_ERR_ARG;
  cudaSetDevice(c->device); c->err.clear();
  int ms = 0;
  TRY(c, refine_local_maxspan(c, &ms));
  *maxspan = ms;
  return 0;
}

int bkid_shard_set_maxspan(bkid_ctx *c, int32_t maxspan) { if (!c) return BKID_ERR_ARG; c->maxspan = maxspan; return 0; }

int bkid_shard_coverage(bkid_ctx *c, double dist, uint32_t **dev_cov, int64_t *n)
{
  if (!c) return BKID_ERR_ARG;
  cudaSetDevice(c->device); c->err.clear();
  TRY(c, refine_coverage(c, dist));
  *dev_cov = c->cov.as<uint32_t>(); *n = 2 * c->n_clusters;
  return 0;
}

int bkid_shard_vote(bkid_ctx *c)
{
  if (!c) return BKID_ERR_ARG;
  cudaSetDevice(c->device); c->err.clear();
  TRY(c, refine_vote(c));
  return sync_check(c);
}

int bkid_shard_depth(bkid_ctx *c, uint32_t **dev_depth, int64_t *n)
{
  if (!c) return BKID_ERR_ARG;
  cudaSetDevice(c->device); c->err.clear();
  TRY(c, refine_depth(c));
  TRY(c, sync_check(c));
  *dev_depth = c->depth.as<uint32_t>(); *n = 2 * c->n_clusters;
  return 0;
}

int bkid_shard_finish(bkid_ctx *c, int64_t *n_called)
// ... 307 lines not shown
```

breakid_b200/csrc/bkid_core.cu:

```cuda
#include "../../include/breakid_b200.h"
#include "prims.cuh"

#include <algorithm>
#include <array>
#include <cmath>
#include <cstdio>
#include <chrono>
#include <cstring>
#include <memory>
#include <map>
#include <string>
#include <vector>

thread_local long long g_bk_launches = 0;
static thread_local std::string g_last_cuda_err;
static std::string g_create_err;

bool g_bk_prof_on = false;
namespace {
struct ProfRec { const char *name; cudaEvent_t e0, e1; };
std::vector<ProfRec> g_prof_recs;
std::vector<cudaEvent_t> g_prof_pool;
cudaEvent_t prof_event()
{
  if (!g_prof_pool.empty()) { cudaEvent_t e = g_prof_pool.back(); g_prof_pool.pop_back(); return e; }
  cudaEvent_t e; cudaEventCreate(&e); return e;
}
}
void bk_prof_begin(const char *name, cudaStream_t st)
{
  ProfRec r{name, prof_event(), prof_event()};
  cudaEventRecord(r.e0, st);
  g_prof_recs.push_back(r);
}
void bk_prof_end(cudaStream_t st) { if (!g_prof_recs.empty()) cudaEventRecord(g_prof_recs.back().e1, st); }

void bk_set_cuda_error(cudaError_t e, const char *file, int line)
{
  char buf[256];
  snprintf(buf, sizeof buf, "CUDA error %d (%s) at %s:%d", (int)e, cudaGetErrorString(e), file, line);
  g_last_cuda_err = buf;
}

using bk::div_up;

enum { F_PAIRED = 0x1, F_PROPER = 0x2, F_UNMAP = 0x4, F_REVERSE = 0x10, F_SECONDARY = 0x100, F_QCFAIL = 0x200, F_DUP = 0x400 };
enum { CL_INSERT = 1, CL_CAND = 2, CL_DEPTH = 4, CL_SPLITOK = 8, CL_EXCL = 16  };

struct DBuf {
  void *p = nullptr;
  size_t cap = 0;
  template <typename T> T *as() const { return (T *)p; }
  int ensure(size_t bytes, size_t keep, cudaStream_t st)
  {
    if (bytes <= cap) return 0;
    size_t ncap = std::max(bytes, cap + cap / 2);
    ncap = (ncap + 255) & ~(size_t)255;
    void *q = nullptr;
    cudaError_t e = cudaMalloc(&q, ncap);
    if (e != cudaSuccess) { bk_set_cuda_error(e, __FILE__, __LINE__); return e == cudaErrorMemoryAllocation ? BKID_ERR_NOMEM : BKID_ERR_CUDA; }
    if (p && keep) cudaMemcpyAsync(q, p, keep, cudaMemcpyDeviceToDevice, st);
    if (p) { cudaStreamSynchronize(st); cudaFree(p); }
    p = q; cap = ncap;
    return 0;
  }
  void release() { if (p) cudaFree(p); p = nullptr; cap = 0; }
};

#define BK_TRY(x) do { int rc__ = (x); if (rc__ != 0) return rc__; } while (0)

constexpr int K1_THREADS = 256;
constexpr int K1_TILE = 4096;
enum { G_SUM = 0, G_CNT = 1, G_SQ = 2, G_CAND = 3, G_XMAX = 4, G_SPAN = 5 };

__device__ __forceinline__ unsigned classify_one(unsigned flag, unsigned mapq, int qual)
{
  unsigned c = 0;
  if ((flag & F_PAIRED) && (flag & F_PROPER) && !(flag & (F_UNMAP | F_SECONDARY | F_QCFAIL | F_DUP))) c |= CL_INSERT;
  if ((int)mapq >= qual && !(flag & F_DUP) && !(flag & F_SECONDARY) && (flag & F_PAIRED) && !(flag & F_PROPER)) c |= CL_CAND;
  if (mapq > 0 && !(flag & F_DUP) && (flag & F_PAIRED)) c |= CL_DEPTH;
  if (!(flag & F_DUP) && (flag & F_PAIRED)) c |= CL_SPLITOK;
  return c;
}

struct ISizeCol {
  const int32_t *w; const int16_t *h;
  __device__ __forceinline__ int at(long long i) const { return h ? (int)h[i] : w[i]; }
};

__device__ __forceinline__ unsigned classify4(unsigned f01, unsigned f23, unsigned m4, unsigned q4, bool q_never, unsigned &ins8)
{
  unsigned ins_lo = __vcmpeq2(f01 & 0x07070707u, 0x00030003u), ins_hi = __vcmpeq2(f23 & 0x07070707u, 0x00030003u);
  unsigned bas_lo = __vcmpeq2(f01 & 0x04010401u, 0x00010001u), bas_hi = __vcmpeq2(f23 & 0x04010401u, 0x00010001u);
  unsigned cnd_lo = __vcmpeq2(f01 & 0x05030503u, 0x00010001u), cnd_hi = __vcmpeq2(f23 & 0x05030503u, 0x00010001u);
  ins8 = __byte_perm(ins_lo, ins_hi, 0x6420);
  unsigned bas8 = __byte_perm(bas_lo, bas_hi, 0x6420), cnd8 = __byte_perm(cnd_lo, cnd_hi, 0x6420);
  unsigned ge8 = q_never ? 0u : __vcmpgeu4(m4, q4), gt8 = __vcmpne4(m4, 0u);
  cnd8 &= ge8;
  return (ins8 & 0x01010101u) | (cnd8 & 0x02020202u) | (bas8 & gt8 & 0x04040404u) | (bas8 & 0x08080808u);
}

template <bool I16, bool S16>
__global__ void __launch_bounds__(K1_THREADS)
k1_classify(const uint16_t *__restrict__ flag, const uint8_t *__restrict__ mapq, const int32_t *__restrict__ isize, const int16_t *__restrict__ isize16,
            const uint16_t *__restrict__ span16, long long n, int qual, uint8_t *__restrict__ cls, uint8_t *__restrict__ cand_bits ,
            unsigned long long *__restrict__ g)
{
  __shared__ unsigned long long sh_sum, sh_sq, sh_cnt, sh_cand;
  __shared__ unsigned sh_xmax, sh_span;
  if (threadIdx.x == 0) { sh_sum = 0; sh_sq = 0; sh_cnt = 0; sh_cand = 0; sh_xmax = 0; sh_span = 0; }
  __syncthreads();
  unsigned long long sum_abs = 0, sum_sq = 0;
  unsigned long long cnt_ins = 0, cnt_cand = 0;
  unsigned xmax = 0, smax2 = 0;
  const unsigned q4 = (unsigned)(qual < 0 ? 0 : (qual > 255 ? 255 : qual)) * 0x01010101u;
  const bool q_never = qual > 255;
  const long long ntiles = (n + K1_TILE - 1) / K1_TILE;
  for (long long tile = blockIdx.x; tile < ntiles; tile += gridDim.x) {
  const long long tile0 = tile * K1_TILE;
  unsigned cnt = 0;
#pragma unroll
  for (int gq = 0; gq < 2; ++gq) {
    long long i = tile0 + gq * (K1_THREADS * 8) + threadIdx.x * 8;
    if (i + 7 < n) {
      uint4 f8 = *reinterpret_cast<const uint4 *>(flag + i);
      uint2 m8 = *reinterpret_cast<const uint2 *>(mapq + i);
      unsigned insA, insB;
      unsigned cA = classify4(f8.x, f8.y, m8.x, q4, q_never, insA), cB = classify4(f8.z, f8.w, m8.y, q4, q_never, insB);
      *reinterpret_cast<uint2 *>(cls + i) = make_uint2(cA, cB);
      {
        unsigned a = (cA >> 1) & 0x01010101u, b = (cB >> 1) & 0x01010101u;
        a = (a | (a >> 7) | (a >> 14) | (a >> 21)) & 0xfu; b = (b | (b >> 7) | (b >> 14) | (b >> 21)) & 0xfu;
        cand_bits[i >> 3] = (uint8_t)(a | (b << 4));
      }
      cnt += __popc(cA & 0x01010101u) + __popc(cB & 0x01010101u) + ((__popc(cA & 0x02020202u) + __popc(cB & 0x02020202u)) << 16);
      if (S16) {
        uint4 p8 = *reinterpret_cast<const uint4 *>(span16 + i);
        smax2 = __vmaxu2(__vmaxu2(smax2, p8.x), __vmaxu2(__vmaxu2(p8.y, p8.z), p8.w));
      }
      if (I16) {
        uint4 s8 = *reinterpret_cast<const uint4 *>(isize16 + i);
        unsigned w[4] = {s8.x, s8.y, s8.z, s8.w};
        unsigned mk[4] = {__byte_perm(insA, 0, 0x1100), __byte_perm(insA, 0, 0x3322), __byte_perm(insB, 0, 0x1100), __byte_perm(insB, 0, 0x3322)};
#pragma unroll
        for (int q = 0; q < 4; ++q) {
          unsigned a2 = __vabs2(w[q]) & mk[q];
          unsigned lo = a2 & 0xffffu, hi = a2 >> 16;
          sum_abs += lo + hi;
          sum_sq += (unsigned long long)lo * lo + (unsigned long long)hi * hi;
          xmax = max(xmax, max(lo, hi));
        }
      } else {
        int4 sA = *reinterpret_cast<const int4 *>(isize + i), sB = *reinterpret_cast<const int4 *>(isize + i + 4);
        int sv[8] = {sA.x, sA.y, sA.z, sA.w, sB.x, sB.y, sB.z, sB.w};
#pragma unroll
        for (int q = 0; q < 8; ++q) {
          unsigned mk = (unsigned)((int)(((q < 4 ? insA : insB) << (24 - 8 * (q & 3)))) >> 31);
          unsigned a = (unsigned)(sv[q] < 0 ? -sv[q] : sv[q]) & mk;
          sum_abs += a; sum_sq += (unsigned long long)a * a; xmax = max(xmax, a);
        }
      }
    } else {
      unsigned tail_bits = 0;
      for (int k = 0; k < 8; ++k)
        if (i + k < n) {
          unsigned c = classify_one(flag[i + k], mapq[i + k], qual);
          if (c & CL_INSERT) {
            int sv = I16 ? (int)isize16[i + k] : isize[i + k];
            unsigned a = (unsigned)(sv < 0 ? -sv : sv);
            sum_abs += a; sum_sq += (unsigned long long)a * a; xmax = max(xmax, a); cnt += 1u;
          }
          if (S16) smax2 = __vmaxu2(smax2, (unsigned)span16[i + k]);
          cnt += ((c >> 1) & 1u) << 16;
          cls[i + k] = (uint8_t)c;
          tail_bits |= ((c >> 1) & 1u) << k;
        }
      if (i < n) cand_bits[i >> 3] = (uint8_t)tail_bits;
    }
  }
  cnt_ins += cnt & 0xffffu; cnt_cand += cnt >> 16;
  }
  unsigned smax = max(smax2 & 0xffffu, smax2 >> 16);
  cnt_ins = bk::warp_sum(cnt_ins); cnt_cand = bk::warp_sum(cnt_cand);
  sum_abs = bk::warp_sum(sum_abs);
  sum_sq = bk::warp_sum(sum_sq);
  for (int o = 16; o; o >>= 1) { xmax = max(xmax, __shfl_xor_sync(0xffffffffu, xmax, o)); smax = max(smax, __shfl_xor_sync(0xffffffffu, smax, o)); }
  if ((threadIdx.x & 31) == 0) { atomicAdd(&sh_cnt, cnt_ins); atomicAdd(&sh_cand, cnt_cand); atomicAdd(&sh_sum, sum_abs); atomicAdd(&sh_sq, sum_sq); atomicMax(&sh_xmax, xmax); atomicMax(&sh_span, smax); }
  __syncthreads();
  if (threadIdx.x == 0) {
    if (sh_cnt) { atomicAdd(g + G_SUM, sh_sum); atomicAdd(g + G_CNT, sh_cnt); atomicAdd(g + G_SQ, sh_sq); atomicMax(g + G_XMAX, (unsigned long long)sh_xmax); }
    if (sh_cand) atomicAdd(g + G_CAND, sh_cand);
    if (S16 && sh_span) atomicMax(g + G_SPAN, (unsigned long long)sh_span);
  }
}

__device__ __forceinline__ long long ex_lower_bound(const int32_t *__restrict__ tid, const int32_t *__restrict__ pos, long long n, int qt, long long qp)
{
  long long lo = 0, hi = n;
  while (lo < hi) {
    long long m = (lo + hi) >> 1;
    uint32_t tm = (uint32_t)tid[m];
    bool less = tm < (uint32_t)qt || (tm == (uint32_t)qt && (long long)pos[m] < qp);
    if (less) lo = m + 1; else hi = m;
  }
  return lo;
}
__global__ void ex_ranges(const int32_t *__restrict__ tid, const int32_t *__restrict__ pos, long long n, const int32_t *__restrict__ iv , int n_iv,
                          uint32_t *__restrict__ lo, uint32_t *__restrict__ len)
{
  int k = blockIdx.x * blockDim.x + threadIdx.x;
  if (k >= n_iv) return;
  long long a = ex_lower_bound(tid, pos, n, iv[3 * k], iv[3 * k + 1]);
  long long b = ex_lower_bound(tid, pos, n, iv[3 * k], iv[3 * k + 2]);
  lo[k] = (uint32_t)a; len[k] = (uint32_t)(b > a ? b - a : 0);
}
__global__ void ex_prefix(const uint32_t *__restrict__ len, int n_iv, unsigned long long *__restrict__ pre )
{
  if (blockIdx.x || threadIdx.x) return;
  unsigned long long s = 0;
  for (int k = 0; k < n_iv; ++k) { pre[k] = s; s += len[k]; }
  pre[n_iv] = s;
}
__global__ void __launch_bounds__(256)
ex_apply(const uint32_t *__restrict__ lo, const unsigned long long *__restrict__ pre, int n_iv, ISizeCol isz, uint8_t *__restrict__ cls, uint8_t *__restrict__ cand_bits,
         unsigned long long *__restrict__ g)
{
  unsigned long long E = pre[n_iv];
  unsigned long long sum = 0, sq = 0; unsigned cnt = 0, ncand = 0;
  for (unsigned long long e = (unsigned long long)blockIdx.x * blockDim.x + threadIdx.x; e < E; e += (unsigned long long)gridDim.x * blockDim.x) {
    int a = 0, b = n_iv;
    while (b - a > 1) { int m = (a + b) >> 1; if (pre[m] <= e) a = m; else b = m; }
    long long i = (long long)lo[a] + (long long)(e - pre[a]);
    unsigned c = cls[i];
    if (c & CL_INSERT) { int s = isz.at(i); unsigned long long x = (unsigned long long)(s < 0 ? -(long long)s : (long long)s); sum += x; sq += x * x; ++cnt; }
    if (c & CL_CAND) { ++ncand; atomicAnd(reinterpret_cast<unsigned *>(cand_bits + ((i >> 3) & ~3ll)), ~(1u << (unsigned)(((i >> 3) & 3ll) * 8 + (i & 7)))); }
    cls[i] = (uint8_t)CL_EXCL;
  }
  sum = bk::warp_sum(sum); sq = bk::warp_sum(sq); cnt = bk::warp_sum(cnt); ncand = bk::warp_sum(ncand);
  if ((threadIdx.x & 31) == 0) {
    if (cnt) { atomicAdd(g + G_SUM, 0ull - sum); atomicAdd(g + G_CNT, 0ull - (unsigned long long)cnt); atomicAdd(g + G_SQ, 0ull - sq); }
    if (ncand) atomicAdd(g + G_CAND, 0ull - (unsigned long long)ncand);
  }
}

constexpr int SD_BLOCK = 8192;
constexpr int SD_THREADS = 256;
constexpr int SD_K = 52;

__device__ __forceinline__ int binade_of(double s)
{
  if (!(s >= 1.0)) return -1;
  return (int)((__double_as_longlong(s) >> 52) & 0x7ff) - 1023;
}

__device__ __forceinline__ void sd_elem(int isz, double mean, double &a, long long &fa, unsigned &kmin)
{
  double x = (double)(isz < 0 ? -isz : isz);
  double d = __dsub_rn(x, mean);
  a = __dmul_rn(d, d);
  double fl = floor(a);
  fa = (long long)fl;
  double frac = a - fl;
  kmin = 255u;
  if (frac >= 0.5) {
    double om = 1.0 - frac;
    long long b = __double_as_longlong(om);
    int e = (int)((b >> 52) & 0x7ff) - 1023;
    int ce = e + ((b & 0xFFFFFFFFFFFFFll) != 0 ? 1 : 0);
    int km = 53 + ce;
    if (km < 0) km = 0;
    if (km < SD_K) kmin = (unsigned)km;
  }
}

constexpr int SD_LUT = 65536;
__device__ __noinline__ unsigned long long sd_entry_slow(int isz, double mean)
{
  double a; long long fa; unsigned km;
  sd_elem(isz, mean, a, fa, km);
  return ((unsigned long long)km << 56) | ((unsigned long long)fa & 0x00ffffffffffffffull);
}
__global__ void sd_build_lut(double mean, unsigned long long *__restrict__ lut)
{
  int x = blockIdx.x * blockDim.x + threadIdx.x;
  if (x >= SD_LUT) return;
  double a; long long fa; unsigned km;
  sd_elem(x, mean, a, fa, km);
  lut[x] = ((unsigned long long)km << 56) | ((unsigned long long)fa & 0x00ffffffffffffffull);
}

__global__ void __launch_bounds__(SD_THREADS)
sd_block_stats(const uint8_t *__restrict__ cls, ISizeCol isz, long long n, double mean, const unsigned long long *__restrict__ lut,
               long long *__restrict__ blkF, uint32_t *__restrict__ blkCum , uint32_t *__restrict__ blkN, double *__restrict__ blkAmax)
{
  __shared__ unsigned hist[SD_K];
  __shared__ unsigned long long sh64[33];
  __shared__ unsigned sh32[33];
  __shared__ double shd[33];
  if (threadIdx.x < SD_K) hist[threadIdx.x] = 0;
  __syncthreads();
  long long base = (long long)blockIdx.x * SD_BLOCK;
  unsigned long long F = 0, famax = 0;
  unsigned cnt = 0;
  unsigned hot = 0;
  for (int g = 0; g < SD_BLOCK / (SD_THREADS * 4); ++g) {
    long long i = base + (long long)g * (SD_THREADS * 4) + threadIdx.x * 4;
    unsigned char c[4];
    int s[4];
    if (i + 3 < n) {
      uchar4 c4 = *reinterpret_cast<const uchar4 *>(cls + i);
      c[0] = c4.x; c[1] = c4.y; c[2] = c4.z; c[3] = c4.w;
      if (isz.h) { short4 h4 = *reinterpret_cast<const short4 *>(isz.h + i); s[0] = h4.x; s[1] = h4.y; s[2] = h4.z; s[3] = h4.w; }
      else { int4 s4 = *reinterpret_cast<const int4 *>(isz.w + i); s[0] = s4.x; s[1] = s4.y; s[2] = s4.z; s[3] = s4.w; }
    } else {
      for (int k = 0; k < 4; ++k) { c[k] = (i + k < n) ? cls[i + k] : 0; s[k] = (i + k < n) ? isz.at(i + k) : 0; }
    }
#pragma unroll
    for (int k = 0; k < 4; ++k) {
      if (c[k] & CL_INSERT) {
        unsigned x = (unsigned)(s[k] < 0 ? -s[k] : s[k]);
        unsigned long long e = (x < (unsigned)SD_LUT) ? __ldg(lut + x) : sd_entry_slow(s[k], mean);
        unsigned long long fa = e & 0x00ffffffffffffffull;
        unsigned km = (unsigned)(e >> 56);
        F += fa;
        ++cnt;
        famax = fa > famax ? fa : famax;
        hot += (km == 51u ? 1u : 0u) + (km == 50u ? (1u << 10) : 0u) + (km == 49u ? (1u << 20) : 0u);
        if (km < 49u) atomicAdd(&hist[km], 1u);
      }
    }
  }
  hot = bk::warp_sum(hot);
  if ((threadIdx.x & 31) == 0) {
    unsigned h51 = hot & 1023u, h50 = (hot >> 10) & 1023u, h49 = hot >> 20;
    if (h51) atomicAdd(&hist[51], h51);
    if (h50) atomicAdd(&hist[50], h50);
    if (h49) atomicAdd(&hist[49], h49);
  }
  double amax = (double)(famax + 1);
  unsigned long long totF;
  bk::block_excl_scan<unsigned long long>(F, sh64, totF);
  unsigned totN;
  bk::block_excl_scan<unsigned>(cnt, sh32, totN);
  for (int o = 16; o; o >>= 1) amax = fmax(amax, __shfl_xor_sync(0xffffffffu, amax, o));
  if ((threadIdx.x & 31) == 0) shd[threadIdx.x >> 5] = amax;
  __syncthreads();
  if (threadIdx.x == 0) {
    double m = 0.0;
    for (int w = 0; w < SD_THREADS / 32; ++w) m = fmax(m, shd[w]);
    blkAmax[blockIdx.x] = m;
    blkF[blockIdx.x] = (long long)totF;
    blkN[blockIdx.x] = totN;
  }
  if (threadIdx.x < 64) {
    unsigned k = threadIdx.x;
    unsigned v = k < SD_K ? hist[k] : 0u;
    unsigned inc = bk::warp_incl_scan(v);
    if (k == 31) sh32[0] = inc;
    __syncwarp();
    if (k < 32) blkCum[(size_t)blockIdx.x * SD_K + k] = inc;
    else sh32[1 + (k - 32)] = inc;
  }
  __syncthreads();
  if (threadIdx.x >= 32 && threadIdx.x < SD_K) blkCum[(size_t)blockIdx.x * SD_K + threadIdx.x] = sh32[0] + sh32[1 + (threadIdx.x - 32)];
}

constexpr int SDR_T = 1024;
__global__ void __launch_bounds__(SDR_T)
sd_resolve(const uint8_t *__restrict__ cls, ISizeCol isz, long long n, double mean, int nb,
           const long long *__restrict__ blkF, const uint32_t *__restrict__ blkCum, const uint32_t *__restrict__ blkN,
           const double *__restrict__ blkAmax, long long t_in, long long *__restrict__ out)
{
  extern __shared__ unsigned char dyn[];
  double *sa = reinterpret_cast<double *>(dyn);
  unsigned char *skm = dyn + (size_t)SD_BLOCK * 8;
  __shared__ long long sh_scan[33];
  __shared__ long long sh_t;
  __shared__ int sh_j, sh_q, sh_oor, sh_k;
  if (threadIdx.x == 0) { sh_t = t_in; sh_j = 0; sh_oor = 0; }
  __syncthreads();
  constexpr int PB = 8;
  while (true) {
    int j0 = sh_j;
    long long t0 = sh_t;
    if (j0 >= nb || sh_oor) break;
    int k0 = binade_of((double)t0);
    int jb = j0 + (int)threadIdx.x * PB;
    long long dl[PB];
    long long delta = 0;
#pragma unroll
    for (int i = 0; i < PB; ++i) {
      int j = jb + i;
      long long v = 0;
      if (j < nb) {
        v = blkF[j];
        if (k0 >= 0 && k0 < SD_K) v += blkCum[(size_t)j * SD_K + k0];
      }
      dl[i] = v; delta += v;
    }
    long long tot;
    long long tstart = t0 + bk::block_excl_scan<long long>(delta, sh_scan, tot);
    int first_bad = SDR_T * PB;
    long long tend_of[PB];
    {
      long long ts = tstart;
#pragma unroll
      for (int i = 0; i < PB; ++i) {
        int j = jb + i;
        bool valid = true;
        if (j < nb) {
          unsigned bn = blkN[j];
          double upper = (double)(ts + dl[i] + (long long)bn + 2) + blkAmax[j] * 1.000000001 + 2.0;
          valid = (bn == 0) || (k0 < SD_K && binade_of((double)ts) == k0 && binade_of(upper) == k0);
          if (bn != 0 && k0 >= SD_K) valid = false;
          if (!valid && first_bad == SDR_T * PB) first_bad = (int)threadIdx.x * PB + i;
        }
        ts += dl[i];
        tend_of[i] = ts;
      }
    }
    if (threadIdx.x == 0) sh_q = SDR_T * PB;
    __syncthreads();
    if (first_bad < SDR_T * PB) atomicMin(&sh_q, first_bad);
    __syncthreads();
    int q = sh_q;
    int nvalid = min(q, nb - j0);
    __syncthreads();
    if (nvalid > 0 && (nvalid - 1) / PB == (int)threadIdx.x) {
      long long te = tend_of[0];
#pragma unroll
      for (int i = 1; i < PB; ++i) if ((nvalid - 1) % PB == i) te = tend_of[i];
      sh_t = te; sh_j = j0 + nvalid;
    }
    __syncthreads();
    if (q >= SDR_T * PB || j0 + q >= nb) continue;
    int jq = j0 + q;
    long long t = sh_t;
    {
      double upper = (double)(t + blkF[jq] + (long long)blkN[jq] + 2) + blkAmax[jq] * 1.000000001 + 2.0;
      int ka = binade_of((double)t), kb = binade_of(upper);
      if (ka == kb && ka < SD_K && q > 0) continue;
    }
    long long base = (long long)jq * SD_BLOCK;
    int m = (int)min((long long)SD_BLOCK, n - base);
    for (int e = threadIdx.x; e < SD_BLOCK; e += SDR_T) {
      double a = -1.0; unsigned km = 255u;
      if (e < m && (cls[base + e] & CL_INSERT)) { long long fa; sd_elem(isz.at(base + e), mean, a, fa, km); }
      sa[e] = a; skm[e] = (unsigned char)km;
    }
    __syncthreads();
    constexpr int PER = SD_BLOCK / SDR_T;
    int p = 0;
    while (p < m) {
      if (threadIdx.x == 0) sh_q = SD_BLOCK;
      __syncthreads();
      {
        int lo = threadIdx.x * PER, best = SD_BLOCK;
        for (int e = lo + PER - 1; e >= lo; --e) if (e >= p && e < m && sa[e] >= 0.0) best = e;
        if (best < SD_BLOCK) atomicMin(&sh_q, best);
      }
      __syncthreads();
      int pe = sh_q;
      if (pe >= SD_BLOCK) break;
      __syncthreads();
      if (threadIdx.x == 0) { sh_k = binade_of((double)t + sa[pe]); sh_q = SD_BLOCK; }
      __syncthreads();
      int k = sh_k;
      if (k >= SD_K) { if (threadIdx.x == 0) sh_oor = 1; __syncthreads(); break; }
      int lo = threadIdx.x * PER;
      long long loc = 0;
      for (int e = lo; e < lo + PER; ++e)
        if (e >= pe && e < m && sa[e] >= 0.0) loc += (long long)floor(sa[e]) + ((k >= 0 && skm[e] <= k) ? 1 : 0);
      long long tt;
      long long run = t + bk::block_excl_scan<long long>(loc, sh_scan, tt);
      int cross = SD_BLOCK;
      for (int e = lo; e < lo + PER; ++e)
        if (e >= pe && e < m && sa[e] >= 0.0) {
          if (e > pe && binade_of((double)run + sa[e]) > k && cross == SD_BLOCK) cross = e;
          run += (long long)floor(sa[e]) + ((k >= 0 && skm[e] <= k) ? 1 : 0);
        }
      if (cross < SD_BLOCK) atomicMin(&sh_q, cross);
      __syncthreads();
      int qx = sh_q;
      long long part = 0;
      for (int e = lo; e < lo + PER; ++e)
        if (e >= pe && e < qx && e < m && sa[e] >= 0.0) part += (long long)floor(sa[e]) + ((k >= 0 && skm[e] <= k) ? 1 : 0);
      long long ptot;
      bk::block_excl_scan<long long>(part, sh_scan, ptot);
      t += ptot;
      p = qx;
      __syncthreads();
    }
    if (threadIdx.x == 0) { sh_t = t; sh_j = jq + 1; }
    __syncthreads();
  }
  if (threadIdx.x == 0) { out[0] = sh_t; out[1] = sh_oor; }
}

__global__ void sd_sequential(const uint8_t *__restrict__ cls, ISizeCol isz, long long n, double mean, long long t_in, long long *out)
{
  if (blockIdx.x || threadIdx.x) return;
  long long t = t_in;
  for (long long i = 0; i < n; ++i)
    if (cls[i] & CL_INSERT) {
      int s = isz.at(i);
      double x = (double)(s < 0 ? -s : s);
      double d = __dsub_rn(x, mean);
      t = (long long)__dadd_rn((double)t, __dmul_rn(d, d));
    }
  out[0] = t; out[1] = 0;
}

__device__ __forceinline__ unsigned long long sd_fast_eval(unsigned x, double mean, double thr, bool &rare, bool &oor)
{
  const double M52 = 4503599627370496.0;
  double xd = __dsub_rn(__hiloint2double(0x43300000, (int)x), M52);
  double d = __dsub_rn(xd, mean);
  double a = __dmul_rn(d, d);
  double sft = __dadd_rd(a, M52);
  double fr = __dsub_rn(a, __dsub_rn(sft, M52));
  rare = fr >= thr;
  oor = !(a < 2251799813685248.0);
  return (unsigned long long)__double_as_longlong(sft) & 0xFFFFFFFFFFFFFull;
}
constexpr int SDF_WIN = 4096;
template <bool NARROW>
__global__ void __launch_bounds__(256)
sd_fast(const uint8_t *__restrict__ cls, const int32_t *__restrict__ isize, const int16_t *__restrict__ isize16, long long n, double mean, double thr,
        unsigned long long *__restrict__ out)
{
  __shared__ uint32_t tab[SDF_WIN + 2];
  const double mc = mean < 0.0 ? 0.0 : (mean > 2.0e9 ? 2.0e9 : mean);
  const unsigned xlo = (unsigned)mc > (unsigned)(SDF_WIN / 2) ? (unsigned)mc - (unsigned)(SDF_WIN / 2) : 0u;
  for (int k = threadIdx.x; k < SDF_WIN; k += blockDim.x) {
    bool rare, oor;
    unsigned long long fa = sd_fast_eval(xlo + (unsigned)k, mean, thr, rare, oor);
    tab[k] = (rare || oor || fa >= (1ull << 28)) ? 0xffffffffu : (uint32_t)fa;
  }
  if (threadIdx.x == 0) { tab[SDF_WIN] = 0xffffffffu; tab[SDF_WIN + 1] = 0u; }
  __syncthreads();
  unsigned long long F = 0; unsigned E = 0, oorf = 0;
  const long long ngroups = (n + 7) / 8;
  for (long long gi = (long long)blockIdx.x * blockDim.x + threadIdx.x; gi < ngroups; gi += (long long)gridDim.x * blockDim.x) {
    long long i = gi * 8;
    unsigned cm;
    int sv[8];
    if (i + 7 < n) {
      uint2 c8 = *reinterpret_cast<const uint2 *>(cls + i);
      cm = (c8.x & 0x01010101u) | ((c8.y & 0x01010101u) << 1);
      if (NARROW) {
        uint4 h8 = *reinterpret_cast<const uint4 *>(isize16 + i);
        sv[0] = (int)(short)(h8.x & 0xffffu); sv[1] = (int)h8.x >> 16; sv[2] = (int)(short)(h8.y & 0xffffu); sv[3] = (int)h8.y >> 16;
        sv[4] = (int)(short)(h8.z & 0xffffu); sv[5] = (int)h8.z >> 16; sv[6] = (int)(short)(h8.w & 0xffffu); sv[7] = (int)h8.w >> 16;
      } else {
        int4 a4 = *reinterpret_cast<const int4 *>(isize + i), b4 = *reinterpret_cast<const int4 *>(isize + i + 4);
        sv[0] = a4.x; sv[1] = a4.y; sv[2] = a4.z; sv[3] = a4.w; sv[4] = b4.x; sv[5] = b4.y; sv[6] = b4.z; sv[7] = b4.w;
      }
    } else {
      cm = 0;
      for (int k = 0; k < 8; ++k) {
        bool on = i + k < n && (cls[i + k] & CL_INSERT);
        sv[k] = (i + k < n) ? (NARROW ? (int)isize16[i + k] : isize[i + k]) : 0;
        if (on) cm |= k < 4 ? (1u << (8 * k)) : (2u << (8 * (k - 4)));
      }
    }
    unsigned part = 0;
#pragma unroll
    for (int k = 0; k < 8; ++k) {
      const unsigned bit = k < 4 ? (1u << (8 * k)) : (2u << (8 * (k - 4)));
      unsigned x = (unsigned)(sv[k] < 0 ? -sv[k] : sv[k]);
      unsigned w = min(x - xlo, (unsigned)SDF_WIN);
      uint32_t t = tab[(cm & bit) ? w : (unsigned)(SDF_WIN + 1)];
      if (t != 0xffffffffu) part += t;
      else {
        bool rare, oor;
        F += sd_fast_eval(x, mean, thr, rare, oor);
        E += rare ? 1u : 0u; oorf |= oor ? 1u : 0u;
      }
    }
    F += part;
  }
  F = bk::warp_sum(F); E = bk::warp_sum(E); oorf = bk::warp_sum(oorf);
  if ((threadIdx.x & 31) == 0) {
    if (F) atomicAdd(out, F);
    if (E) atomicAdd(out + 1, (unsigned long long)E);
    if (oorf) atomicOr(out + 2, 1ull);
  }
}

__device__ __forceinline__ long long x_slot_of(const uint32_t *__restrict__ x_rec, long long n_x, uint32_t i)
{
  long long lo = 0, hi = n_x;
  while (lo < hi) { long long m = (lo + hi) >> 1; if (x_rec[m] < i) lo = m + 1; else hi = m; }
  return (lo < n_x && x_rec[lo] == i) ? lo : -1;
}

constexpr int KX_THREADS = 256;
constexpr int KX_ITEMS = 2;
constexpr int KX_TILE = KX_THREADS * KX_ITEMS;

__global__ void __launch_bounds__(KX_THREADS) kx_count(const uint32_t *__restrict__ x_rec, long long n_x, const uint8_t *__restrict__ cand_bits, long long n,
                                                       uint32_t *__restrict__ tile_cnt, uint8_t *__restrict__ is_cand , int *__restrict__ bad)
{
  __shared__ unsigned sh32[33];
  long long j0 = (long long)blockIdx.x * KX_TILE + threadIdx.x * KX_ITEMS;
  unsigned cnt = 0, bits = 0;
  uint32_t r[KX_ITEMS]; unsigned char c[KX_ITEMS];
  uint32_t rprev = j0 > 0 && j0 < n_x ? x_rec[j0 - 1] : 0u;
#pragma unroll
  for (int k = 0; k < KX_ITEMS; ++k) r[k] = j0 + k < n_x ? x_rec[j0 + k] : 0xffffffffu;
#pragma unroll
  for (int k = 0; k < KX_ITEMS; ++k)
    c[k] = (j0 + k < n_x && (long long)r[k] < n) ? (unsigned char)(((cand_bits[r[k] >> 3] >> (r[k] & 7u)) & 1u) ? CL_CAND : 0) : 0;
#pragma unroll
  for (int k = 0; k < KX_ITEMS; ++k) {
    long long j = j0 + k;
    if (j < n_x) {
      if ((long long)r[k] >= n || (j > 0 && rprev >= r[k])) atomicExch(bad, 1);
      else if (c[k] & CL_CAND) { ++cnt; bits |= 1u << k; }
      rprev = r[k];
    }
  }
  if (j0 < n_x) is_cand[j0 / KX_ITEMS] = (uint8_t)bits;
  unsigned tot;
  bk::block_excl_scan<unsigned>(cnt, sh32, tot);
  if (threadIdx.x == 0) tile_cnt[blockIdx.x] = tot;
}

__global__ void __launch_bounds__(KX_THREADS) kx_write(const uint32_t *__restrict__ x_rec, long long n_x, const uint8_t *__restrict__ is_cand, long long n, const uint32_t *__restrict__ tile_off,
                                                       const uint16_t *__restrict__ flag, const uint8_t *__restrict__ mapq, const int32_t *__restrict__ tid, const int32_t *__restrict__ pos,
                                                       const int32_t *__restrict__ x_mtid, const int32_t *__restrict__ x_mpos, const uint64_t *__restrict__ x_nh,
                                                       unsigned long long index_offset, bkid_cand *__restrict__ out, uint64_t *__restrict__ keys, uint32_t *__restrict__ vals)
{
  __shared__ unsigned sh32[33];
  long long j0 = (long long)blockIdx.x * KX_TILE + threadIdx.x * KX_ITEMS;
  __shared__ __align__(16) bkid_cand srow[KX_TILE];
  const unsigned bits = j0 < n_x ? (unsigned)is_cand[j0 / KX_ITEMS] : 0u;
  unsigned tot;
  unsigned loc = bk::block_excl_scan<unsigned>(__popc(bits), sh32, tot);
  const unsigned tile0 = tile_off[blockIdx.x];
  uint32_t i4[KX_ITEMS]; int32_t t4[KX_ITEMS], p4[KX_ITEMS]; uint16_t f4[KX_ITEMS]; uint8_t m4[KX_ITEMS];
#pragma unroll
  for (int k = 0; k < KX_ITEMS; ++k) i4[k] = (bits >> k) & 1u ? x_rec[j0 + k] : 0u;
#pragma unroll
  for (int k = 0; k < KX_ITEMS; ++k)
    if ((bits >> k) & 1u) { t4[k] = tid[i4[k]]; p4[k] = pos[i4[k]]; f4[k] = flag[i4[k]]; m4[k] = mapq[i4[k]]; }
#pragma unroll
  for (int k = 0; k < KX_ITEMS; ++k)
    if ((bits >> k) & 1u) {
      long long j = j0 + k;
      bkid_cand c;
      c.name_lo = x_nh[2 * (size_t)j]; c.name_hi = x_nh[2 * (size_t)j + 1];
      c.tid = t4[k]; c.pos = p4[k]; c.mtid = x_mtid[j]; c.mpos = x_mpos[j];
      c.gidx = index_offset + i4[k];
      c.flag = f4[k]; c.mapq = m4[k];
      c._pad[0] = c._pad[1] = c._pad[2] = c._pad[3] = c._pad[4] = 0;
      srow[loc++] = c;
    }
  __syncthreads();
  const uint4 *sv = reinterpret_cast<const uint4 *>(srow);
  uint4 *ov = reinterpret_cast<uint4 *>(out + tile0);
  for (unsigned i = threadIdx.x; i < tot * 3u; i += KX_THREADS) ov[i] = sv[i];
  if (keys)
    for (unsigned i = threadIdx.x; i < tot; i += KX_THREADS) { keys[tile0 + i] = srow[i].name_lo; vals[tile0 + i] = tile0 + i; }
}

__global__ void k2_cand_keys(const bkid_cand *__restrict__ cand, long long nc, uint64_t *__restrict__ keys, uint32_t *__restrict__ vals)
{
  long long p = (long long)blockIdx.x * blockDim.x + threadIdx.x;
  if (p < nc) { keys[p] = cand[p].name_lo; vals[p] = (uint32_t)p; }
}

__device__ __forceinline__ uint32_t genome_pos(const uint32_t *__restrict__ cum, int nt, int tid, int pos)
{
  uint32_t p = (tid > 0) ? cum[tid < nt ? tid : nt] : 0u;
  return p + (uint32_t)pos;
}

constexpr int PAIR_IDX_BITS = 40;
constexpr uint32_t NO_MATE = 0xffffffffu;

__device__ __forceinline__ bool pair_is_discordant(const bkid_cand &I, const bkid_cand &J, double w)
{
  int ti = I.tid < 0 ? -1 : I.tid, tj = J.tid < 0 ? -1 : J.tid;
  long long pi = (long long)I.pos + 1, pj = (long long)J.pos + 1;
  long long dp = pi - pj; if (dp < 0) dp = -dp;
  return (ti != tj) || ((double)dp >= w);
}
__device__ __forceinline__ bkid_pair make_pair(const bkid_cand &I, const bkid_cand &J, const uint32_t *__restrict__ cum, int nt, const int32_t *__restrict__ bucket_rank)
{
  uint32_t c1 = genome_pos(cum, nt, I.tid, I.pos);
  uint32_t c2 = genome_pos(cum, nt, I.mtid, I.mpos);
  bkid_pair P;
  P.name_lo = I.name_lo; P.name_hi = I.name_hi;
  int ti = I.tid < 0 ? -1 : I.tid, tj = J.tid < 0 ? -1 : J.tid;
  uint32_t pi = (uint32_t)((long long)I.pos + 1), pj = (uint32_t)((long long)J.pos + 1);
  if (c1 <= c2) {
    P.p1_flag = I.flag; P.p1_tid = ti; P.p1_pos = pi; P.p1_mapq = I.mapq;
    P.p2_flag = J.flag; P.p2_tid = tj; P.p2_pos = pj; P.p2_mapq = J.mapq;
    P.p1_chr_pos = c1; P.p2_chr_pos = c2;
  } else {
    P.p2_flag = I.flag; P.p2_tid = ti; P.p2_pos = pi; P.p2_mapq = I.mapq;
    P.p1_flag = J.flag; P.p1_tid = tj; P.p1_pos = pj; P.p1_mapq = J.mapq;
    P.p1_chr_pos = c2; P.p2_chr_pos = c1;
  }
  P.p1_strand = (P.p1_flag & F_REVERSE) ? '-' : '+';
  P.p2_strand = (P.p2_flag & F_REVERSE) ? '-' : '+';
  int a = P.p1_tid + 1, b = P.p2_tid + 1;
  P.bucket = bucket_rank[a * (nt + 1) + b];
  P.cluster = -1;
  P.orig = (uint32_t)(I.gidx & 0xffffffffull);
  P._pad = (uint32_t)((I.gidx >> 32) & 0xffull);
  return P;
}

__global__ void __launch_bounds__(256) k2_join(uint64_t *__restrict__ keys, uint32_t *__restrict__ vals, const uint32_t *__restrict__ nc_dev, uint32_t nc_host,
                                               const bkid_cand *__restrict__ cand, int group_bits, uint32_t cap, double w, uint32_t *__restrict__ mate, int *__restrict__ too_big)
{
  const uint32_t nc = nc_dev ? *nc_dev : nc_host;
  uint32_t p = blockIdx.x * blockDim.x + threadIdx.x;
  if (p >= nc) return;
  const uint64_t gmask = group_bits >= 64 ? ~0ull : ((1ull << group_bits) - 1ull);
  const uint64_t k0 = keys[p], gk = k0 & gmask;
  if (p > 0 && (keys[p - 1] & gmask) == gk) return;
  uint32_t e = p + 1;
  while (e < nc && (keys[e] & gmask) == gk) ++e;
  if (e - p < 2) return;
  uint64_t hi_prev = cand[vals[p]].name_hi;
  bool mixed = false;
  for (uint32_t q = p + 1; q < e && !mixed; ++q) mixed = keys[q] != k0 || cand[vals[q]].name_hi != hi_prev;
  if (mixed) {
    if (e - p > cap) { atomicExch(too_big, 1); return; }
    for (uint32_t i = p + 1; i < e; ++i) {
      uint64_t kl = keys[i]; uint32_t v = vals[i]; uint64_t kh = cand[v].name_hi;
      uint32_t j = i;
      while (j > p) {
        uint64_t pl = keys[j - 1], ph = cand[vals[j - 1]].name_hi;
        if (pl < kl || (pl == kl && ph <= kh)) break;
// ... 596 lines not shown
```

breakid_b200/csrc/bkid_dist.cuh:

```cuda
#pragma once
#include <condition_variable>
#include <dlfcn.h>
#include <mutex>
#include <thread>

enum BkOp { BK_SUM = 0, BK_MAX = 1 };
enum BkType { BK_U32 = 0, BK_U64 = 1 };

struct bkid_comm {
  int rank = 0, world = 1;
  std::string err;
  virtual ~bkid_comm() {}
  virtual int allreduce(void *dev, int n, BkType ty, BkOp op, cudaStream_t st) = 0;
  virtual int allgather_host(const uint64_t *mine, int n, uint64_t *all) = 0;
  virtual int alltoallv(const void *send, const uint64_t *send_off, void *recv, const uint64_t *recv_off, int row_bytes, cudaStream_t st) = 0;
  virtual int allgatherv(const void *send, uint64_t nrows, void *recv, const uint64_t *recv_off, int row_bytes, cudaStream_t st) = 0;
  virtual int relay_i64(long long *v, int from, int to) = 0;
  virtual void abort() {}
};

struct LocalGroup {
  int world;
  std::mutex mu; std::condition_variable cv; int arrived = 0; unsigned long long gen = 0;
  bool aborted = false;
// ... 186 lines not shown

template <int MODE>
__global__ void __launch_bounds__(RT_THREADS) rt_count(const void *__restrict__ rows, long long n, uint32_t W, const uint8_t *__restrict__ table, uint32_t *__restrict__ tile_cnt , int ntiles)
{
  __shared__ unsigned h[RT_MAXW];
  if (threadIdx.x < RT_MAXW) h[threadIdx.x] = 0;
  __syncthreads();
  long long i = (long long)blockIdx.x * RT_THREADS + threadIdx.x;
  unsigned o = i < n ? row_owner<MODE>(rows, i, W, table) : 0xffffffffu;
  unsigned m = __match_any_sync(0xffffffffu, o);
  if (i < n && (threadIdx.x & 31) == (unsigned)(__ffs(m) - 1)) atomicAdd(&h[o], (unsigned)__popc(m));
  __syncthreads();
  if (threadIdx.x < W) tile_cnt[(size_t)threadIdx.x * ntiles + blockIdx.x] = h[threadIdx.x];
}

template <int MODE>
__global__ void __launch_bounds__(RT_THREADS) rt_scatter(const void *__restrict__ rows, long long n, uint32_t W, const uint8_t *__restrict__ table, const uint32_t *__restrict__ tile_off ,
                                                         int ntiles, int row_chunks , uint4 *__restrict__ out)
{
  __shared__ unsigned wcnt[RT_THREADS / 32][RT_MAXW];
  const unsigned w = threadIdx.x >> 5, l = threadIdx.x & 31;
  for (int k = threadIdx.x; k < (RT_THREADS / 32) * RT_MAXW; k += RT_THREADS) (&wcnt[0][0])[k] = 0;
  __syncthreads();
  long long i = (long long)blockIdx.x * RT_THREADS + threadIdx.x;
  unsigned o = i < n ? row_owner<MODE>(rows, i, W, table) : 0xffffffffu;
  unsigned m = __match_any_sync(0xffffffffu, o);
  unsigned before = __popc(m & ((1u << l) - 1u));
  if (i < n && before == 0) wcnt[w][o] = (unsigned)__popc(m);
  __syncthreads();
  if (i >= n) return;
  unsigned base = tile_off[(size_t)o * ntiles + blockIdx.x];
  for (unsigned ww = 0; ww < w; ++ww) base += wcnt[ww][o];
  const uint4 *src = reinterpret_cast<const uint4 *>(rows) + i * row_chunks;
  uint4 *dst = out + (size_t)(base + before) * row_chunks;
  for (int k = 0; k < row_chunks; ++k) dst[k] = src[k];
}

__global__ void pair_bucket_hist(const bkid_pair *__restrict__ pairs, long long n, unsigned *__restrict__ hist)
{
  long long i = (long long)blockIdx.x * blockDim.x + threadIdx.x;
  if (i < n) atomicAdd(&hist[pairs[i].bucket], 1u);
}
__global__ void rows_sorted_check(const bkid_sarow *__restrict__ rows, long long n, int *__restrict__ bad)
{
  long long i = (long long)blockIdx.x * blockDim.x + threadIdx.x;
  if (i + 1 >= n) return;
  const EvRow &a = reinterpret_cast<const EvRow *>(rows)[i], &b = reinterpret_cast<const EvRow *>(rows)[i + 1];
  uint32_t ta = (uint32_t)a.tid, tb = (uint32_t)b.tid;
  if (ta > tb || (ta == tb && a.pos > b.pos)) atomicExch(bad, 1);
}
__global__ void cluster_bucket_dense(bkid_cluster_rec *cl, uint32_t n, const int32_t *__restrict__ ranks, int nranks)
{
  uint32_t i = blockIdx.x * blockDim.x + threadIdx.x;
  if (i >= n) return;
  int a = 0, b = nranks;
  int v = cl[i].bucket;
  while (a < b) { int m = (a + b) >> 1; if (ranks[m] < v) a = m + 1; else b = m; }
  cl[i].bucket = a;
}

template <int MODE>
static int route_rows(bkid_ctx *c, const void *rows, long long n, int row_bytes, uint32_t W, const uint8_t *table, DBuf &out, std::vector<uint64_t> &send_off)
{
  cudaStream_t st = c->st;
  send_off.assign(W + 1, 0);
  TRY(c, out.ensure((size_t)std::max<long long>(n, 1) * row_bytes, 0, st));
  if (n <= 0) return 0;
  int ntiles = div_up(n, RT_THREADS);
  size_t cells = (size_t)W * ntiles;
  TRY(c, c->sc.ensure((long long)cells + 8, st));
  uint32_t *cnt = c->sc.a32.as<uint32_t>(), *off = c->sc.b32.as<uint32_t>();
  BK_LAUNCH((rt_count<MODE>), ntiles, RT_THREADS, 0, st, rows, n, W, table, cnt, ntiles);
  bk::exclusive_scan<uint32_t, uint32_t>(cnt, off, (long long)cells, c->sc.scan_tmp.as<unsigned long long>(), nullptr, st);
  BK_LAUNCH((rt_scatter<MODE>), ntiles, RT_THREADS, 0, st, rows, n, W, table, off, ntiles, row_bytes / 16, out.as<uint4>());
  std::vector<uint32_t> h(W);
  for (uint32_t r = 0; r < W; ++r) CU(c, cudaMemcpyAsync(&h[r], off + (size_t)r * ntiles, 4, cudaMemcpyDeviceToHost, st));
  TRY(c, sync_check(c));
  for (uint32_t r = 0; r < W; ++r) send_off[r] = h[r];
  send_off[W] = (uint64_t)n;
  return 0;
}

static int exchange_rows(bkid_ctx *c, bkid_comm *cm, const DBuf &send, const std::vector<uint64_t> &send_off, int row_bytes, DBuf &recv, long long *n_recv)
{
  int W = cm->world;
  std::vector<uint64_t> cnt(W), all((size_t)W * W), recv_off(W + 1, 0);
  for (int r = 0; r < W; ++r) cnt[r] = send_off[r + 1] - send_off[r];
  if (cm->allgather_host(cnt.data(), W, all.data())) return fail(c, BKID_ERR_CUDA, "count exchange failed: " + cm->err);
  for (int s = 0; s < W; ++s) recv_off[s + 1] = recv_off[s] + all[(size_t)s * W + cm->rank];
  TRY(c, recv.ensure((size_t)std::max<uint64_t>(recv_off[W], 1) * row_bytes, 0, c->st));
  if (cm->alltoallv(send.p, send_off.data(), recv.p, recv_off.data(), row_bytes, c->st)) return fail(c, BKID_ERR_CUDA, "all-to-all failed: " + cm->err);
  *n_recv = (long long)recv_off[W];
  return 0;
}

static int gather_rows_all(bkid_ctx *c, bkid_comm *cm, const void *mine, long long n_mine, int row_bytes, DBuf &recv, long long *n_all)
{
  int W = cm->world;
  uint64_t k = (uint64_t)n_mine;
  std::vector<uint64_t> all(W), off(W + 1, 0);
  if (cm->allgather_host(&k, 1, all.data())) return fail(c, BKID_ERR_CUDA, "count exchange failed: " + cm->err);
  for (int s = 0; s < W; ++s) off[s + 1] = off[s] + all[s];
  TRY(c, recv.ensure((size_t)std::max<uint64_t>(off[W], 1) * row_bytes, 0, c->st));
  if (cm->allgatherv(mine, k, recv.p, off.data(), row_bytes, c->st)) return fail(c, BKID_ERR_CUDA, "all-gather failed: " + cm->err);
  *n_all = (long long)off[W];
  return 0;
}

static void lpt_owner_table(const std::vector<unsigned long long> &hist, int W, std::vector<uint8_t> &owner)
{
  std::vector<int> order;
  for (int b = 0; b < (int)hist.size(); ++b) if (hist[b]) order.push_back(b);
  std::stable_sort(order.begin(), order.end(), [&](int a, int b) { return hist[a] > hist[b]; });
  std::vector<double> load(W, 0.0);
  owner.assign(hist.size(), 0);
  for (int b : order) {
    int best = 0;
    for (int r = 1; r < W; ++r) if (load[r] < load[best]) best = r;
    owner[b] = (uint8_t)best;
    double m = (double)hist[b];
    load[best] += m * (1.0 + log2(m + 1.0) / 16.0);
  }
}

struct DistTimes { float stats = 0, candidates = 0, a2a_cand = 0, join = 0, a2a_pairs = 0, cluster = 0, gather = 0, refine = 0, total = 0; };

static int dist_run_impl(bkid_ctx *c, bkid_comm *cm, int mode, double *mean_o, double *sd_o, double *dist_o, int64_t *n_called, DistTimes *tmo)
{
  const int W = cm->world, R = cm->rank;
  cudaSetDevice(c->device);
  c->err.clear();
  cudaStream_t st = c->st;
  auto now = [] { return std::chrono::steady_clock::now(); };
  auto ms_since = [](std::chrono::steady_clock::time_point t0) { return std::chrono::duration<float, std::milli>(std::chrono::steady_clock::now() - t0).count(); };
  auto T0 = now(), t0 = T0;
  DistTimes tm;
  if (W > RT_MAXW) return fail(c, BKID_ERR_ARG, "more than 32 ranks");
  TRY(c, classify_impl(c));
  TRY(c, c->dist_scalars.ensure(4096, 0, st));
  unsigned long long *dv = c->dist_scalars.as<unsigned long long>();
  unsigned long long hv[4] = {(unsigned long long)c->sum_abs, (unsigned long long)c->cnt_insert, c->sum_sq, (unsigned long long)c->n};
  CU(c, cudaMemcpyAsync(dv, hv, 32, cudaMemcpyHostToDevice, st));
  if (cm->allreduce(dv, 3, BK_U64, BK_SUM, st)) return fail(c, BKID_ERR_CUDA, "all-reduce failed: " + cm->err);
  unsigned long long xm = c->xmax;
  CU(c, cudaMemcpyAsync(dv + 8, &xm, 8, cudaMemcpyHostToDevice, st));
  if (cm->allreduce(dv + 8, 1, BK_U64, BK_MAX, st)) return fail(c, BKID_ERR_CUDA, "all-reduce failed: " + cm->err);
  unsigned long long gs[3], gxm;
  CU(c, cudaMemcpyAsync(gs, dv, 24, cudaMemcpyDeviceToHost, st)); CU(c, cudaMemcpyAsync(&gxm, dv + 8, 8, cudaMemcpyDeviceToHost, st));
  TRY(c, sync_check(c));
  const unsigned long long S = gs[0], N = gs[1], SQ = gs[2];
  const double mean = (double)(long long)S / (double)(long long)N;
  const int kub = sd_upper_binade(S, N, SQ, gxm);
  const long long local_insert = c->cnt_insert;
  TRY(c, sd_fast_launch(c, mean, kub, c->st2));
  std::vector<uint64_t> ns(W);
  { uint64_t mine = (uint64_t)c->n; if (cm->allgather_host(&mine, 1, ns.data())) return fail(c, BKID_ERR_CUDA, "count exchange failed: " + cm->err); }
  unsigned long long offset = 0;
  for (int r = 0; r < R; ++r) offset += ns[r];
  tm.stats = ms_since(t0); t0 = now();
  TRY(c, extract_candidates(c, offset, false));
  {
    unsigned hnc[2] = {0, 0};
    CU(c, cudaMemcpyAsync(hnc, c->counters.as<unsigned>() + CS_NC, 8, cudaMemcpyDeviceToHost, st));
    TRY(c, sync_check(c));
    TRY(c, check_candidates(c, hnc));
  }
  tm.candidates = ms_since(t0); t0 = now();
  std::vector<uint64_t> soff;
  TRY(c, route_rows<0>(c, c->cand.p, c->n_cand, (int)sizeof(bkid_cand), (uint32_t)W, nullptr, c->dist_send, soff));
  long long nc_all = 0;
  TRY(c, exchange_rows(c, cm, c->dist_send, soff, (int)sizeof(bkid_cand), c->dist_recv, &nc_all));
  tm.a2a_cand = ms_since(t0); t0 = now();
  unsigned long long F = 0, E = 0;
  TRY(c, sd_fast_collect(c, c->st2, &F, &E));
  unsigned long long fe[2] = {F, E == ~0ull ? (1ull << 40) : std::min<unsigned long long>(E, 1ull << 40)};
  if (local_insert <= 0) { fe[0] = 0; fe[1] = 0; }
  CU(c, cudaMemcpyAsync(dv + 16, fe, 16, cudaMemcpyHostToDevice, st));
  if (cm->allreduce(dv + 16, 2, BK_U64, BK_SUM, st)) return fail(c, BKID_ERR_CUDA, "all-reduce failed: " + cm->err);
  CU(c, cudaMemcpyAsync(fe, dv + 16, 16, cudaMemcpyDeviceToHost, st));
  TRY(c, sync_check(c));
  long long total = (long long)fe[0];
  if (fe[1] != 0 && N > 0) {
    TRY(c, sd_prepare_impl(c, mean));
    long long t = 0;
    for (int src = 0; src < W; ++src) {
      if (R == src) { long long tout = t; TRY(c, sd_partial_impl(c, mean, t, &tout)); t = tout; }
      if (src + 1 < W && cm->relay_i64(&t, src, src + 1)) return fail(c, BKID_ERR_CUDA, "sd relay failed: " + cm->err);
    }
    unsigned long long tv = R == W - 1 ? (unsigned long long)t : 0ull;
    CU(c, cudaMemcpyAsync(dv + 24, &tv, 8, cudaMemcpyHostToDevice, st));
    if (cm->allreduce(dv + 24, 1, BK_U64, BK_SUM, st)) return fail(c, BKID_ERR_CUDA, "all-reduce failed: " + cm->err);
    CU(c, cudaMemcpyAsync(&tv, dv + 24, 8, cudaMemcpyDeviceToHost, st));
    TRY(c, sync_check(c));
    total = (long long)tv;
  }
  const double sd = sqrt((double)total / (double)(long long)N);
  const int times = c->prm.times;
  const double d = times * sqrt((double)times) * (mean + c->prm.sd_mult * sd);
  c->mean = mean; c->sd = sd; c->have_stats = true;
  long long np = 0;
  TRY(c, join_candidates(c, c->dist_recv.as<bkid_cand>(), nc_all, d, &np));
  tm.join = ms_since(t0); t0 = now();
  const int nbk = (c->nt + 1) * (c->nt + 1);
  TRY(c, c->tmpF.ensure((size_t)nbk * 8 + 64, 0, st));
  unsigned *bh = c->tmpF.as<unsigned>();
  CU(c, cudaMemsetAsync(bh, 0, (size_t)nbk * 4, st));
  if (np > 0) BK_LAUNCH(pair_bucket_hist, GRID1(np, 256), 256, 0, st, c->pairs_tmp.as<bkid_pair>(), np, bh);
  if (cm->allreduce(bh, nbk, BK_U32, BK_SUM, st)) return fail(c, BKID_ERR_CUDA, "all-reduce failed: " + cm->err);
  std::vector<unsigned> hb(nbk);
  CU(c, cudaMemcpyAsync(hb.data(), bh, (size_t)nbk * 4, cudaMemcpyDeviceToHost, st));
  TRY(c, sync_check(c));
  std::vector<unsigned long long> hist(hb.begin(), hb.end());
  std::vector<uint8_t> owner;
  lpt_owner_table(hist, W, owner);
  uint8_t *d_owner = (uint8_t *)(bh + nbk);
  CU(c, cudaMemcpyAsync(d_owner, owner.data(), (size_t)nbk, cudaMemcpyHostToDevice, st));
  TRY(c, route_rows<1>(c, c->pairs_tmp.p, np, (int)sizeof(bkid_pair), (uint32_t)W, d_owner, c->dist_send, soff));
  long long np_all = 0;
  TRY(c, exchange_rows(c, cm, c->dist_send, soff, (int)sizeof(bkid_pair), c->dist_recv, &np_all));
  tm.a2a_pairs = ms_since(t0); t0 = now();
  TRY(c, set_pairs(c, c->dist_recv.as<bkid_pair>(), np_all, false));
  c->tm.n_pairs = c->np0;
  c->scanned = true; c->clustered = c->refined = false;
  int64_t ncl_local = 0;
  TRY(c, bkid_cluster(c, d, mode, &ncl_local));
  tm.cluster = ms_since(t0); t0 = now();
  const bkid_cluster_rec *cl_dev = nullptr; int64_t ncl_mine = 0;
  TRY(c, bkid_shard_clusters(c, &cl_dev, &ncl_mine));
  long long ncl_all = 0;
  TRY(c, gather_rows_all(c, cm, cl_dev, ncl_mine, (int)sizeof(bkid_cluster_rec), c->dist_recv, &ncl_all));
  {
    std::vector<bkid_cluster_rec> hcl((size_t)std::max<long long>(ncl_all, 1));
    if (ncl_all) CU(c, cudaMemcpyAsync(hcl.data(), c->dist_recv.p, (size_t)ncl_all * sizeof(bkid_cluster_rec), cudaMemcpyDeviceToHost, st));
    TRY(c, sync_check(c));
    hcl.resize((size_t)ncl_all);
    std::stable_sort(hcl.begin(), hcl.end(), [](const bkid_cluster_rec &a, const bkid_cluster_rec &b) { return a.bucket != b.bucket ? a.bucket < b.bucket : a.id < b.id; });
    TRY(c, c->clusters.ensure((size_t)(ncl_all + 1) * sizeof(bkid_cluster_rec), 0, st));
    if (ncl_all) CU(c, cudaMemcpyAsync(c->clusters.p, hcl.data(), (size_t)ncl_all * sizeof(bkid_cluster_rec), cudaMemcpyHostToDevice, st));
    TRY(c, sync_check(c));
    c->n_clusters = ncl_all; c->clusters_ranked = true; c->clustered = true; c->refined = false;
  }
  std::vector<int32_t> all_ranks;
  {
    int64_t nbl = c->nb;
    long long nb_all = 0;
    TRY(c, gather_rows_all(c, cm, c->bucket_rank_of.p, nbl, 4, c->dist_send, &nb_all));
    all_ranks.resize((size_t)nb_all);
    if (nb_all) CU(c, cudaMemcpyAsync(all_ranks.data(), c->dist_send.p, (size_t)nb_all * 4, cudaMemcpyDeviceToHost, st));
    TRY(c, sync_check(c));
    std::sort(all_ranks.begin(), all_ranks.end());
  }
  TRY(c, refine_build_rows(c));
  long long nrows_all = 0;
  TRY(c, gather_rows_all(c, cm, c->sarows.p, c->n_sa, (int)sizeof(bkid_sarow), c->dist_rows, &nrows_all));
  {
    int *bad = (int *)(c->counters.as<unsigned>() + CS_MISSING);
    CU(c, cudaMemsetAsync(bad, 0, 4, st));
    if (nrows_all > 1) BK_LAUNCH(rows_sorted_check, GRID1(nrows_all, 256), 256, 0, st, (const bkid_sarow *)c->dist_rows.p, nrows_all, bad);
    int hbad = 0;
    CU(c, cudaMemcpyAsync(&hbad, bad, 4, cudaMemcpyDeviceToHost, st));
    TRY(c, sync_check(c));
    if (hbad) return fail(c, BKID_ERR_ARG, "the ranks' record slices are not in coordinate order (rank r must hold the r-th genomic bin)");
  }
  c->rows_ptr = c->dist_rows.p; c->n_rows = nrows_all;
  tm.gather = ms_since(t0); t0 = now();
  c->n_called = 0;
  if (ncl_all > 0) {
    int ms_local = 0;
    TRY(c, refine_local_maxspan(c, &ms_local));
    unsigned long long msv = (unsigned long long)ms_local;
    CU(c, cudaMemcpyAsync(dv + 32, &msv, 8, cudaMemcpyHostToDevice, st));
    if (cm->allreduce(dv + 32, 1, BK_U64, BK_MAX, st)) return fail(c, BKID_ERR_CUDA, "all-reduce failed: " + cm->err);
    CU(c, cudaMemcpyAsync(&msv, dv + 32, 8, cudaMemcpyDeviceToHost, st));
    TRY(c, sync_check(c));
    c->maxspan = (int)msv;
    TRY(c, refine_coverage(c, d));
    if (cm->allreduce(c->cov.p, (int)(2 * ncl_all), BK_U32, BK_SUM, st)) return fail(c, BKID_ERR_CUDA, "all-reduce failed: " + cm->err);
    TRY(c, refine_vote(c));
    TRY(c, refine_depth(c));
    if (cm->allreduce(c->depth.p, (int)(2 * ncl_all), BK_U32, BK_SUM, st)) return fail(c, BKID_ERR_CUDA, "all-reduce failed: " + cm->err);
    TRY(c, refine_finish(c));
    if (c->n_called > 0 && !all_ranks.empty()) {
      TRY(c, c->tmpF.ensure(all_ranks.size() * 4 + 64, 0, st));
      CU(c, cudaMemcpyAsync(c->tmpF.p, all_ranks.data(), all_ranks.size() * 4, cudaMemcpyHostToDevice, st));
      BK_LAUNCH(cluster_bucket_dense, GRID1(c->n_called, 128), 128, 0, st, c->clusters_out.as<bkid_cluster_rec>(), (uint32_t)c->n_called, c->tmpF.as<int32_t>(), (int)all_ranks.size());
      TRY(c, sync_check(c));
    }
  } else {
  }
  c->refined = true;
  c->tm.n_called = c->n_called;
  tm.refine = ms_since(t0);
  tm.total = ms_since(T0);
  if (mean_o) *mean_o = mean;
  if (sd_o) *sd_o = sd;
  if (dist_o) *dist_o = d;
  if (n_called) *n_called = c->n_called;
  if (tmo) *tmo = tm;
  return 0;
}

extern "C" {

bkid_comm *bkid_comm_nccl_init(const uint8_t *unique_id , int rank, int world, int device)
{
  std::string err;
  if (!g_nccl.load(err)) { g_create_err = err; return nullptr; }
  if (cudaSetDevice(device) != cudaSuccess) { g_create_err = "cudaSetDevice failed"; return nullptr; }
  NcclComm *cm = new NcclComm();
  cm->rank = rank; cm->world = world; cm->device = device;
  NcclApi::uid_t id;
  memcpy(&id, unique_id, sizeof id);
  int rc = g_nccl.CommInitRank(&cm->comm, world, id, rank);
  if (rc != 0) { g_create_err = std::string("ncclCommInitRank: ") + g_nccl.GetErrorString(rc); cm->comm = nullptr; delete cm; return nullptr; }
  return cm;
}

int bkid_comm_nccl_unique_id(uint8_t *out )
{
  std::string err;
  if (!g_nccl.load(err)) { g_create_err = err; return BKID_ERR_CUDA; }
  NcclApi::uid_t id;
  int rc = g_nccl.GetUniqueId(&id);
  if (rc != 0) { g_create_err = std::string("ncclGetUniqueId: ") + g_nccl.GetErrorString(rc); return BKID_ERR_CUDA; }
  memcpy(out, &id, sizeof id);
  return 0;
}
// ... 59 lines not shown
```

Before: 52.98 billion.

## Build insert-size histogram in classify and compute SD sum from histogram

The classify kernel now also builds a 65536-bin histogram of absolute insert sizes. It uses per-warp shared-memory windows centred on each tile's first insert value and falls back to global atomics outside them. The exclusion kernel subtracts excluded rows from that histogram. The SD fast pass, which used to stream the whole cls and isize columns again, now evaluates each histogram bin once and weights it by the count. This removes a full pass over the data but adds shared-memory atomics and extra shared memory to the hot classify kernel. Inputs with very large insert sizes fall back to the general path.

Result: slower. 51.85 billion (median of 6 runs) (-2.1%).

```diff
diff --git a/breakid_b200/csrc/bkid_api.cuh b/breakid_b200/csrc/bkid_api.cuh
--- a/breakid_b200/csrc/bkid_api.cuh
+++ b/breakid_b200/csrc/bkid_api.cuh
@@ -56,6 +56,7 @@
   long long n = 0, cap_n = 0;
   bool borrowed = false;
   DBuf flag, mapq, tid, pos, isize, endpos, cls, cand_bits;
+  DBuf ihist;
   DBuf isize16, span16;
   int form_isize = 0, form_span = 0;
   long long reserve_hint = 0;
@@ -80,7 +81,7 @@
   unsigned long long sum_sq = 0, xmax = 0;
   long long n_cand_k1 = 0;
   int sd_kub = 0;
-  bool sd_fast_pending = false;
+  bool sd_hist_pending = false;
   DBuf tile_cand, counters, cand_idx, cand, bucket_rank_of;
   long long n_cand = 0;
   DBuf pairs0, pairs_tmp, bucket_off0;
@@ -587,6 +588,10 @@
   cudaMemset(c->d_nib_len.p, 0, (size_t)(nt + 1) * 8);
   c->nib.resize(nt); c->nib_len.assign(nt, 0);
   cudaFuncSetAttribute(sd_resolve, cudaFuncAttributeMaxDynamicSharedMemorySize, SD_BLOCK * 9);
+  cudaFuncSetAttribute(k1_classify<true, true>, cudaFuncAttributePreferredSharedMemoryCarveout, cudaSharedmemCarveoutMaxShared);
+  cudaFuncSetAttribute(k1_classify<true, false>, cudaFuncAttributePreferredSharedMemoryCarveout, cudaSharedmemCarveoutMaxShared);
+  cudaFuncSetAttribute(k1_classify<false, true>, cudaFuncAttributePreferredSharedMemoryCarveout, cudaSharedmemCarveoutMaxShared);
+  cudaFuncSetAttribute(k1_classify<false, false>, cudaFuncAttributePreferredSharedMemoryCarveout, cudaSharedmemCarveoutMaxShared);
   cudaFuncSetAttribute(is_heap, cudaFuncAttributeMaxDynamicSharedMemorySize, (int)(IS_HEAP_SMEM_ELEMS * 8 + 16));
   cudaFuncSetAttribute(ahc_replay_smem, cudaFuncAttributeMaxDynamicSharedMemorySize, 49 * 4096);
   cudaFuncSetAttribute(ahc_replay_rank, cudaFuncAttributeMaxDynamicSharedMemorySize, 49 * 4096);
@@ -601,7 +606,7 @@
   cudaSetDevice(c->device);
   cudaStreamSynchronize(c->st);
   decoder_free(c);
-  for (DBuf *b : {&c->d_cum, &c->d_bucket_rank, &c->d_canon, &c->flag, &c->mapq, &c->tid, &c->pos, &c->isize, &c->endpos, &c->isize16, &c->span16, &c->cand_bits, &c->x_rec, &c->x_mtid, &c->x_mpos, &c->x_nh, &c->cls,
+  for (DBuf *b : {&c->d_cum, &c->d_bucket_rank, &c->d_canon, &c->flag, &c->mapq, &c->tid, &c->pos, &c->isize, &c->endpos, &c->isize16, &c->span16, &c->cand_bits, &c->ihist, &c->x_rec, &c->x_mtid, &c->x_mpos, &c->x_nh, &c->cls,
                   &c->sa_rec, &c->cig_off, &c->cig_ops, &c->sa_off, &c->sa_txt, &c->oc_off, &c->oc_txt, &c->seq_off, &c->seq4, &c->seq_len, &c->d_nib_ptr, &c->d_nib_len, &c->tile_cand, &c->counters,
                   &c->cand_idx, &c->cand, &c->bucket_rank_of, &c->pairs0, &c->pairs_tmp, &c->bucket_off0, &c->X, &c->Y, &c->bucket_of_pair, &c->cur1, &c->curb1, &c->seg1, &c->mem_pair,
                   &c->mem_bucket, &c->mem_cluster, &c->sdtab, &c->sdlut, &c->clusters, &c->clusters_out, &c->sarows, &c->name_key, &c->name_row, &c->ex_tab, &c->ex_lo, &c->ex_len, &c->ex_pre, &c->work, &c->cov, &c->depth, &c->evoff, &c->valid, &c->tmpA, &c->tmpB, &c->tmpC, &c->tmpD, &c->tmpE, &c->tmpF, &c->tmpG, &c->tmpH, &c->dist_send, &c->dist_recv, &c->dist_rows, &c->dist_scalars, &c->sortbig, &c->sortheap})
@@ -620,7 +625,7 @@
 
 static void invalidate(bkid_ctx *c)
 {
-  if (c->sd_side_pending || c->sd_fast_pending) { cudaStreamSynchronize(c->st2); c->sd_side_pending = false; c->sd_fast_pending = false; }
+  if (c->sd_side_pending || c->sd_hist_pending) { cudaStreamSynchronize(c->st2); c->sd_side_pending = false; c->sd_hist_pending = false; }
   if (c->maxspan_pending) { cudaStreamSynchronize(c->st3); c->maxspan_pending = false; }
   c->classified = c->have_stats = c->scanned = c->clustered = c->refined = false; c->sd_prepared = false; c->maxspan_cached = false;
 }
@@ -899,8 +904,11 @@
   int ntiles = div_up(std::max<long long>(n, 1), K1_TILE);
   TRY(c, c->cls.ensure((size_t)n + 64, 0, st));
   TRY(c, c->cand_bits.ensure((size_t)n / 8 + 64, 0, st));
+  TRY(c, c->ihist.ensure((size_t)IH_BINS * 4, 0, st));
   unsigned long long *g = (unsigned long long *)(c->counters.as<unsigned>() + CS_G);
+  uint32_t *ih = c->ihist.as<uint32_t>();
   CU(c, cudaMemsetAsync(g, 0, 64, st));
+  CU(c, cudaMemsetAsync(ih, 0, (size_t)IH_BINS * 4, st));
   cudaEventRecord(c->ev[2], st);
   const bool i16 = c->p_isize16 != nullptr, s16 = c->p_span16 != nullptr;
   if (n > 0) {
@@ -911,10 +919,10 @@
     else if (s16) cudaOccupancyMaxActiveBlocksPerMultiprocessor(&occ, k1_classify<false, true>, K1_THREADS, 0);
     else cudaOccupancyMaxActiveBlocksPerMultiprocessor(&occ, k1_classify<false, false>, K1_THREADS, 0);
     ntiles = std::min(ntiles, c->n_sm * std::max(occ, 1));
-    if (i16 && s16) BK_LAUNCH((k1_classify<true, true>), (unsigned)ntiles, K1_THREADS, 0, st, c->p_flag, c->p_mapq, c->p_isize, c->p_isize16, c->p_span16, n, c->prm.qual, cls, c->cand_bits.as<uint8_t>(), g);
-    else if (i16) BK_LAUNCH((k1_classify<true, false>), (unsigned)ntiles, K1_THREADS, 0, st, c->p_flag, c->p_mapq, c->p_isize, c->p_isize16, c->p_span16, n, c->prm.qual, cls, c->cand_bits.as<uint8_t>(), g);
-    else if (s16) BK_LAUNCH((k1_classify<false, true>), (unsigned)ntiles, K1_THREADS, 0, st, c->p_flag, c->p_mapq, c->p_isize, c->p_isize16, c->p_span16, n, c->prm.qual, cls, c->cand_bits.as<uint8_t>(), g);
-    else BK_LAUNCH((k1_classify<false, false>), (unsigned)ntiles, K1_THREADS, 0, st, c->p_flag, c->p_mapq, c->p_isize, c->p_isize16, c->p_span16, n, c->prm.qual, cls, c->cand_bits.as<uint8_t>(), g);
+    if (i16 && s16) BK_LAUNCH((k1_classify<true, true>), (unsigned)ntiles, K1_THREADS, 0, st, c->p_flag, c->p_mapq, c->p_isize, c->p_isize16, c->p_span16, n, c->prm.qual, cls, c->cand_bits.as<uint8_t>(), g, ih);
+    else if (i16) BK_LAUNCH((k1_classify<true, false>), (unsigned)ntiles, K1_THREADS, 0, st, c->p_flag, c->p_mapq, c->p_isize, c->p_isize16, c->p_span16, n, c->prm.qual, cls, c->cand_bits.as<uint8_t>(), g, ih);
+    else if (s16) BK_LAUNCH((k1_classify<false, true>), (unsigned)ntiles, K1_THREADS, 0, st, c->p_flag, c->p_mapq, c->p_isize, c->p_isize16, c->p_span16, n, c->prm.qual, cls, c->cand_bits.as<uint8_t>(), g, ih);
+    else BK_LAUNCH((k1_classify<false, false>), (unsigned)ntiles, K1_THREADS, 0, st, c->p_flag, c->p_mapq, c->p_isize, c->p_isize16, c->p_span16, n, c->prm.qual, cls, c->cand_bits.as<uint8_t>(), g, ih);
   }
   cudaEventRecord(c->ev[3], st);
   int n_iv = (int)(c->ex_iv.size() / 3);
@@ -926,7 +934,7 @@
     CU(c, cudaMemcpyAsync(c->ex_tab.p, c->ex_iv.data(), (size_t)n_iv * 12, cudaMemcpyHostToDevice, st));
     BK_LAUNCH(ex_ranges, GRID1(n_iv, 128), 128, 0, st, c->p_tid, c->p_pos, n, c->ex_tab.as<int32_t>(), n_iv, c->ex_lo.as<uint32_t>(), c->ex_len.as<uint32_t>());
     BK_LAUNCH(ex_prefix, 1, 32, 0, st, c->ex_len.as<uint32_t>(), n_iv, c->ex_pre.as<unsigned long long>());
-    BK_LAUNCH(ex_apply, 148 * 8, 256, 0, st, c->ex_lo.as<uint32_t>(), c->ex_pre.as<unsigned long long>(), n_iv, isize_col(c), c->cls.as<uint8_t>(), c->cand_bits.as<uint8_t>(), g);
+    BK_LAUNCH(ex_apply, 148 * 8, 256, 0, st, c->ex_lo.as<uint32_t>(), c->ex_pre.as<unsigned long long>(), n_iv, isize_col(c), c->cls.as<uint8_t>(), c->cand_bits.as<uint8_t>(), g, ih);
     CU(c, cudaMemcpyAsync(&ne, c->ex_pre.as<unsigned long long>() + n_iv, 8, cudaMemcpyDeviceToHost, st));
   }
   unsigned long long h[6] = {0, 0, 0, 0, 0, 0};
@@ -1005,30 +1013,25 @@
   return 0;
 }
 
-static int sd_fast_launch(bkid_ctx *c, double mean, int kub, cudaStream_t st)
-{
-  long long n = c->n;
+static bool sd_hist_covers(const bkid_ctx *c, int kub) { return kub < 51 && c->xmax < (unsigned long long)IH_BINS; }
+static int sd_hist_launch(bkid_ctx *c, double mean, int kub, cudaStream_t st)
+{
   unsigned long long *out = (unsigned long long *)(c->counters.as<unsigned>() + CS_SDF);
   CU(c, cudaMemsetAsync(out, 0, 24, st));
   c->sd_kub = kub;
-  if (n <= 0 || c->cnt_insert <= 0) return 0;
+  if (c->n <= 0 || c->cnt_insert <= 0 || !sd_hist_covers(c, kub)) return 0;
   double thr = 1.0 - ldexp(1.0, kub - 53);
-  int occ = 0;
-  if (c->p_isize16) cudaOccupancyMaxActiveBlocksPerMultiprocessor(&occ, sd_fast<true>, 256, 0);
-  else cudaOccupancyMaxActiveBlocksPerMultiprocessor(&occ, sd_fast<false>, 256, 0);
-  const int grid = c->n_sm * std::max(occ, 1);
-  if (c->p_isize16) BK_LAUNCH((sd_fast<true>), grid, 256, 0, st, c->cls.as<uint8_t>(), c->p_isize, c->p_isize16, n, mean, thr, out);
-  else BK_LAUNCH((sd_fast<false>), grid, 256, 0, st, c->cls.as<uint8_t>(), c->p_isize, c->p_isize16, n, mean, thr, out);
-  return 0;
-}
-static int sd_fast_collect(bkid_ctx *c, cudaStream_t st, unsigned long long *F, unsigned long long *E)
+  BK_LAUNCH(sd_hist, IH_BINS / SDH_THREADS, SDH_THREADS, 0, st, c->ihist.as<uint32_t>(), mean, thr, out);
+  return 0;
+}
+static int sd_hist_collect(bkid_ctx *c, cudaStream_t st, unsigned long long *F, unsigned long long *E)
 {
   unsigned long long h[3] = {0, 0, 0};
   CU(c, cudaMemcpyAsync(h, c->counters.as<unsigned>() + CS_SDF, 24, cudaMemcpyDeviceToHost, st));
   CU(c, cudaStreamSynchronize(st));
   CU(c, cudaGetLastError());
   *F = h[0]; *E = h[2] ? ~0ull : h[1];
-  if (c->sd_kub >= 51 && c->cnt_insert > 0) *E = ~0ull;
+  if (c->cnt_insert > 0 && !sd_hist_covers(c, c->sd_kub)) *E = ~0ull;
   return 0;
 }
 
@@ -1038,9 +1041,9 @@
   long long n = c->n;
   c->mean = (double)c->sum_abs / (double)c->cnt_insert;
   cudaEventRecord(c->ev_side[0], s2);
-  TRY(c, sd_fast_launch(c, c->mean, sd_upper_binade((unsigned long long)c->sum_abs, (unsigned long long)c->cnt_insert, c->sum_sq, c->xmax), s2));
+  TRY(c, sd_hist_launch(c, c->mean, sd_upper_binade((unsigned long long)c->sum_abs, (unsigned long long)c->cnt_insert, c->sum_sq, c->xmax), s2));
   cudaEventRecord(c->ev_side[1], s2);
-  c->sd_fast_pending = true;
+  c->sd_hist_pending = true;
   if (!c->maxspan_cached) {
     int *mx = (int *)(c->counters.as<unsigned>() + CS_MAXSPAN);
     CU(c, cudaMemsetAsync(mx, 0, 4, c->st3));
@@ -1053,8 +1056,8 @@
 static int side_collect(bkid_ctx *c)
 {
   unsigned long long F = 0, E = 0;
-  TRY(c, sd_fast_collect(c, c->st2, &F, &E));
-  c->sd_fast_pending = false;
+  TRY(c, sd_hist_collect(c, c->st2, &F, &E));
+  c->sd_hist_pending = false;
   float ms = 0; cudaEventElapsedTime(&ms, c->ev_side[0], c->ev_side[1]);
   long long total = (long long)F;
   if (E != 0 && c->n > 0 && c->cnt_insert > 0) {
@@ -1096,8 +1099,8 @@
     unsigned long long F = 0, E = 0;
     const bool general_only = getenv("BKID_SD_GENERAL") != nullptr;
     if (!general_only) {
-      TRY(c, sd_fast_launch(c, c->mean, sd_upper_binade((unsigned long long)c->sum_abs, (unsigned long long)c->cnt_insert, c->sum_sq, c->xmax), st));
-      TRY(c, sd_fast_collect(c, st, &F, &E));
+      TRY(c, sd_hist_launch(c, c->mean, sd_upper_binade((unsigned long long)c->sum_abs, (unsigned long long)c->cnt_insert, c->sum_sq, c->xmax), st));
+      TRY(c, sd_hist_collect(c, st, &F, &E));
     }
     long long t = (long long)F;
     if ((general_only || E != 0) && c->n > 0 && c->cnt_insert > 0) TRY(c, sd_partial_impl(c, c->mean, 0, &t));
@@ -1536,8 +1539,8 @@
   if (!c) return BKID_ERR_ARG;
   cudaSetDevice(c->device); c->err.clear();
   TRY(c, classify_impl(c));
-  TRY(c, sd_fast_launch(c, mean, upper_binade, c->st2));
-  c->sd_fast_pending = true;
+  TRY(c, sd_hist_launch(c, mean, upper_binade, c->st2));
+  c->sd_hist_pending = true;
   return 0;
 }
 
@@ -1546,8 +1549,8 @@
   if (!c || !sum_floor || !n_correctable) return BKID_ERR_ARG;
   cudaSetDevice(c->device); c->err.clear();
   unsigned long long F = 0, E = 0;
-  TRY(c, sd_fast_collect(c, c->st2, &F, &E));
-  c->sd_fast_pending = false;
+  TRY(c, sd_hist_collect(c, c->st2, &F, &E));
+  c->sd_hist_pending = false;
   *sum_floor = F; *n_correctable = E == ~0ull ? (uint64_t)1 << 62 : E;
   return 0;
 }
diff --git a/breakid_b200/csrc/bkid_core.cu b/breakid_b200/csrc/bkid_core.cu
--- a/breakid_b200/csrc/bkid_core.cu
+++ b/breakid_b200/csrc/bkid_core.cu
@@ -71,7 +71,27 @@
 
 constexpr int K1_THREADS = 256;
 constexpr int K1_TILE = 4096;
+constexpr int IH_BINS = 65536;
+constexpr int K1_CORE = 256;
+constexpr int K1_WIDE = 2048;
 enum { G_SUM = 0, G_CNT = 1, G_SQ = 2, G_CAND = 3, G_XMAX = 4, G_SPAN = 5 };
+
+__device__ __forceinline__ unsigned ih_window_base(unsigned v, unsigned win)
+{
+  unsigned b = v > win / 2 ? v - win / 2 : 0u;
+  return min(b, (unsigned)IH_BINS - win);
+}
+__device__ __forceinline__ unsigned ih_first_key(bool ins, unsigned v) { return ins && v < (unsigned)IH_BINS ? (threadIdx.x << 16) | v : ~0u; }
+
+__shared__ __align__(16) unsigned k1_win[K1_CORE * 32 + K1_WIDE];
+__device__ __forceinline__ void k1_bin(unsigned v, bool ins, unsigned core_base, unsigned wide_base, uint32_t *__restrict__ hist)
+{
+  if (!ins) return;
+  unsigned o = v - core_base, w = v - wide_base;
+  if (o < (unsigned)K1_CORE) atomicAdd(&k1_win[o * 32 + (threadIdx.x & 31)], 1u);
+  else if (w < (unsigned)K1_WIDE) atomicAdd(&k1_win[K1_CORE * 32 + w], 1u);
+  else if (v < (unsigned)IH_BINS) atomicAdd(hist + v, 1u);
+}
 
 __device__ __forceinline__ unsigned classify_one(unsigned flag, unsigned mapq, int qual)
 {
@@ -104,12 +124,26 @@
 __global__ void __launch_bounds__(K1_THREADS)
 k1_classify(const uint16_t *__restrict__ flag, const uint8_t *__restrict__ mapq, const int32_t *__restrict__ isize, const int16_t *__restrict__ isize16,
             const uint16_t *__restrict__ span16, long long n, int qual, uint8_t *__restrict__ cls, uint8_t *__restrict__ cand_bits ,
-            unsigned long long *__restrict__ g)
+            unsigned long long *__restrict__ g, uint32_t *__restrict__ hist )
 {
   __shared__ unsigned long long sh_sum, sh_sq, sh_cnt, sh_cand;
-  __shared__ unsigned sh_xmax, sh_span;
-  if (threadIdx.x == 0) { sh_sum = 0; sh_sq = 0; sh_cnt = 0; sh_cand = 0; sh_xmax = 0; sh_span = 0; }
+  __shared__ unsigned sh_xmax, sh_span, sh_first;
+  for (int k = threadIdx.x; k < (K1_CORE * 32 + K1_WIDE) / 4; k += K1_THREADS) reinterpret_cast<uint4 *>(k1_win)[k] = make_uint4(0u, 0u, 0u, 0u);
+  if (threadIdx.x == 0) { sh_sum = 0; sh_sq = 0; sh_cnt = 0; sh_cand = 0; sh_xmax = 0; sh_span = 0; sh_first = ~0u; }
   __syncthreads();
+  {
+    long long i = (long long)blockIdx.x * K1_TILE + threadIdx.x;
+    unsigned key = ~0u;
+    if (i < n) {
+      int sv = I16 ? (int)isize16[i] : isize[i];
+      key = ih_first_key(classify_one(flag[i], 0u, 0) & CL_INSERT, sv < 0 ? 0u - (unsigned)sv : (unsigned)sv);
+    }
+    key = __reduce_min_sync(0xffffffffu, key);
+    if ((threadIdx.x & 31) == 0 && key != ~0u) atomicMin(&sh_first, key);
+  }
+  __syncthreads();
+  const unsigned centre = sh_first == ~0u ? 0u : (sh_first & 0xffffu);
+  const unsigned core_base = ih_window_base(centre, K1_CORE), wide_base = ih_window_base(centre, K1_WIDE);
   unsigned long long sum_abs = 0, sum_sq = 0;
   unsigned long long cnt_ins = 0, cnt_cand = 0;
   unsigned xmax = 0, smax2 = 0;
@@ -149,6 +183,8 @@
           sum_abs += lo + hi;
           sum_sq += (unsigned long long)lo * lo + (unsigned long long)hi * hi;
           xmax = max(xmax, max(lo, hi));
+          k1_bin(lo, mk[q] & 1u, core_base, wide_base, hist);
+          k1_bin(hi, mk[q] >> 31, core_base, wide_base, hist);
         }
       } else {
         int4 sA = *reinterpret_cast<const int4 *>(isize + i), sB = *reinterpret_cast<const int4 *>(isize + i + 4);
@@ -158,6 +194,7 @@
           unsigned mk = (unsigned)((int)(((q < 4 ? insA : insB) << (24 - 8 * (q & 3)))) >> 31);
           unsigned a = (unsigned)(sv[q] < 0 ? -sv[q] : sv[q]) & mk;
           sum_abs += a; sum_sq += (unsigned long long)a * a; xmax = max(xmax, a);
+          k1_bin(a, mk != 0u, core_base, wide_base, hist);
         }
       }
     } else {
@@ -169,6 +206,7 @@
             int sv = I16 ? (int)isize16[i + k] : isize[i + k];
             unsigned a = (unsigned)(sv < 0 ? -sv : sv);
             sum_abs += a; sum_sq += (unsigned long long)a * a; xmax = max(xmax, a); cnt += 1u;
+            k1_bin(a, true, core_base, wide_base, hist);
           }
           if (S16) smax2 = __vmaxu2(smax2, (unsigned)span16[i + k]);
           cnt += ((c >> 1) & 1u) << 16;
@@ -187,6 +225,14 @@
   for (int o = 16; o; o >>= 1) { xmax = max(xmax, __shfl_xor_sync(0xffffffffu, xmax, o)); smax = max(smax, __shfl_xor_sync(0xffffffffu, smax, o)); }
   if ((threadIdx.x & 31) == 0) { atomicAdd(&sh_cnt, cnt_ins); atomicAdd(&sh_cand, cnt_cand); atomicAdd(&sh_sum, sum_abs); atomicAdd(&sh_sq, sum_sq); atomicMax(&sh_xmax, xmax); atomicMax(&sh_span, smax); }
   __syncthreads();
+  for (int k = threadIdx.x; k < K1_CORE; k += K1_THREADS) {
+    unsigned s = 0;
+#pragma unroll 8
+    for (int j = 0; j < 32; ++j) s += k1_win[k * 32 + ((j + k) & 31)];
+    if (s) atomicAdd(hist + core_base + k, s);
+  }
+  for (int k = threadIdx.x; k < K1_WIDE; k += K1_THREADS)
+    if (k1_win[K1_CORE * 32 + k]) atomicAdd(hist + wide_base + k, k1_win[K1_CORE * 32 + k]);
   if (threadIdx.x == 0) {
     if (sh_cnt) { atomicAdd(g + G_SUM, sh_sum); atomicAdd(g + G_CNT, sh_cnt); atomicAdd(g + G_SQ, sh_sq); atomicMax(g + G_XMAX, (unsigned long long)sh_xmax); }
     if (sh_cand) atomicAdd(g + G_CAND, sh_cand);
@@ -221,18 +267,44 @@
   for (int k = 0; k < n_iv; ++k) { pre[k] = s; s += len[k]; }
   pre[n_iv] = s;
 }
+constexpr int EX_WIN = 4096;
 __global__ void __launch_bounds__(256)
 ex_apply(const uint32_t *__restrict__ lo, const unsigned long long *__restrict__ pre, int n_iv, ISizeCol isz, uint8_t *__restrict__ cls, uint8_t *__restrict__ cand_bits,
-         unsigned long long *__restrict__ g)
-{
+         unsigned long long *__restrict__ g, uint32_t *__restrict__ hist)
+{
+  __shared__ unsigned sh_win[EX_WIN];
+  __shared__ unsigned sh_first;
+  for (int k = threadIdx.x; k < EX_WIN; k += blockDim.x) sh_win[k] = 0u;
+  if (threadIdx.x == 0) sh_first = ~0u;
+  __syncthreads();
   unsigned long long E = pre[n_iv];
   unsigned long long sum = 0, sq = 0; unsigned cnt = 0, ncand = 0;
-  for (unsigned long long e = (unsigned long long)blockIdx.x * blockDim.x + threadIdx.x; e < E; e += (unsigned long long)gridDim.x * blockDim.x) {
-    int a = 0, b = n_iv;
-    while (b - a > 1) { int m = (a + b) >> 1; if (pre[m] <= e) a = m; else b = m; }
-    long long i = (long long)lo[a] + (long long)(e - pre[a]);
-    unsigned c = cls[i];
-    if (c & CL_INSERT) { int s = isz.at(i); unsigned long long x = (unsigned long long)(s < 0 ? -(long long)s : (long long)s); sum += x; sq += x * x; ++cnt; }
+  unsigned base = 0;
+  bool first = true;
+  for (unsigned long long e0 = (unsigned long long)blockIdx.x * blockDim.x; e0 < E; e0 += (unsigned long long)gridDim.x * blockDim.x) {
+    unsigned long long e = e0 + threadIdx.x;
+    long long i = -1;
+    unsigned c = 0, x = 0;
+    if (e < E) {
+      int a = 0, b = n_iv;
+      while (b - a > 1) { int m = (a + b) >> 1; if (pre[m] <= e) a = m; else b = m; }
+      i = (long long)lo[a] + (long long)(e - pre[a]);
+      c = cls[i];
+      if (c & CL_INSERT) { int s = isz.at(i); x = s < 0 ? 0u - (unsigned)s : (unsigned)s; }
+    }
+    if (first) {
+      unsigned key = __reduce_min_sync(0xffffffffu, ih_first_key(c & CL_INSERT, x));
+      if ((threadIdx.x & 31) == 0 && key != ~0u) atomicMin(&sh_first, key);
+      __syncthreads();
+      base = sh_first == ~0u ? 0u : ih_window_base(sh_first & 0xffffu, EX_WIN);
+      first = false;
+    }
+    if (i < 0) continue;
+    if (c & CL_INSERT) {
+      sum += x; sq += (unsigned long long)x * x; ++cnt;
+      if (x - base < (unsigned)EX_WIN) atomicAdd(sh_win + (x - base), 1u);
+      else if (x < (unsigned)IH_BINS) atomicSub(hist + x, 1u);
+    }
     if (c & CL_CAND) { ++ncand; atomicAnd(reinterpret_cast<unsigned *>(cand_bits + ((i >> 3) & ~3ll)), ~(1u << (unsigned)(((i >> 3) & 3ll) * 8 + (i & 7)))); }
     cls[i] = (uint8_t)CL_EXCL;
   }
@@ -241,6 +313,9 @@
     if (cnt) { atomicAdd(g + G_SUM, 0ull - sum); atomicAdd(g + G_CNT, 0ull - (unsigned long long)cnt); atomicAdd(g + G_SQ, 0ull - sq); }
     if (ncand) atomicAdd(g + G_CAND, 0ull - (unsigned long long)ncand);
   }
+  __syncthreads();
+  for (int k = threadIdx.x; k < EX_WIN; k += blockDim.x)
+    if (sh_win[k]) atomicSub(hist + base + k, sh_win[k]);
 }
 
 constexpr int SD_BLOCK = 8192;
@@ -523,67 +598,22 @@
   oor = !(a < 2251799813685248.0);
   return (unsigned long long)__double_as_longlong(sft) & 0xFFFFFFFFFFFFFull;
 }
-constexpr int SDF_WIN = 4096;
-template <bool NARROW>
-__global__ void __launch_bounds__(256)
-sd_fast(const uint8_t *__restrict__ cls, const int32_t *__restrict__ isize, const int16_t *__restrict__ isize16, long long n, double mean, double thr,
-        unsigned long long *__restrict__ out)
-{
-  __shared__ uint32_t tab[SDF_WIN + 2];
-  const double mc = mean < 0.0 ? 0.0 : (mean > 2.0e9 ? 2.0e9 : mean);
-  const unsigned xlo = (unsigned)mc > (unsigned)(SDF_WIN / 2) ? (unsigned)mc - (unsigned)(SDF_WIN / 2) : 0u;
-  for (int k = threadIdx.x; k < SDF_WIN; k += blockDim.x) {
+constexpr int SDH_THREADS = 256;
+__global__ void __launch_bounds__(SDH_THREADS)
+sd_hist(const uint32_t *__restrict__ hist, double mean, double thr, unsigned long long *__restrict__ out)
+{
+  const unsigned v = blockIdx.x * SDH_THREADS + threadIdx.x;
+  const unsigned h = hist[v];
+  unsigned long long F = 0, E = 0; unsigned oorf = 0;
+  if (h) {
     bool rare, oor;
-    unsigned long long fa = sd_fast_eval(xlo + (unsigned)k, mean, thr, rare, oor);
-    tab[k] = (rare || oor || fa >= (1ull << 28)) ? 0xffffffffu : (uint32_t)fa;
-  }
-  if (threadIdx.x == 0) { tab[SDF_WIN] = 0xffffffffu; tab[SDF_WIN + 1] = 0u; }
-  __syncthreads();
-  unsigned long long F = 0; unsigned E = 0, oorf = 0;
-  const long long ngroups = (n + 7) / 8;
-  for (long long gi = (long long)blockIdx.x * blockDim.x + threadIdx.x; gi < ngroups; gi += (long long)gridDim.x * blockDim.x) {
-    long long i = gi * 8;
-    unsigned cm;
-    int sv[8];
-    if (i + 7 < n) {
-      uint2 c8 = *reinterpret_cast<const uint2 *>(cls + i);
-      cm = (c8.x & 0x01010101u) | ((c8.y & 0x01010101u) << 1);
-      if (NARROW) {
-        uint4 h8 = *reinterpret_cast<const uint4 *>(isize16 + i);
-        sv[0] = (int)(short)(h8.x & 0xffffu); sv[1] = (int)h8.x >> 16; sv[2] = (int)(short)(h8.y & 0xffffu); sv[3] = (int)h8.y >> 16;
-        sv[4] = (int)(short)(h8.z & 0xffffu); sv[5] = (int)h8.z >> 16; sv[6] = (int)(short)(h8.w & 0xffffu); sv[7] = (int)h8.w >> 16;
-      } else {
-        int4 a4 = *reinterpret_cast<const int4 *>(isize + i), b4 = *reinterpret_cast<const int4 *>(isize + i + 4);
-        sv[0] = a4.x; sv[1] = a4.y; sv[2] = a4.z; sv[3] = a4.w; sv[4] = b4.x; sv[5] = b4.y; sv[6] = b4.z; sv[7] = b4.w;
-      }
-    } else {
-      cm = 0;
-      for (int k = 0; k < 8; ++k) {
-        bool on = i + k < n && (cls[i + k] & CL_INSERT);
-        sv[k] = (i + k < n) ? (NARROW ? (int)isize16[i + k] : isize[i + k]) : 0;
-        if (on) cm |= k < 4 ? (1u << (8 * k)) : (2u << (8 * (k - 4)));
-      }
-    }
-    unsigned part = 0;
-#pragma unroll
-    for (int k = 0; k < 8; ++k) {
-      const unsigned bit = k < 4 ? (1u << (8 * k)) : (2u << (8 * (k - 4)));
-      unsigned x = (unsigned)(sv[k] < 0 ? -sv[k] : sv[k]);
-      unsigned w = min(x - xlo, (unsigned)SDF_WIN);
-      uint32_t t = tab[(cm & bit) ? w : (unsigned)(SDF_WIN + 1)];
-      if (t != 0xffffffffu) part += t;
-      else {
-        bool rare, oor;
-        F += sd_fast_eval(x, mean, thr, rare, oor);
-        E += rare ? 1u : 0u; oorf |= oor ? 1u : 0u;
-      }
-    }
-    F += part;
+    F = sd_fast_eval(v, mean, thr, rare, oor) * h;
+    E = rare ? h : 0u; oorf = oor ? 1u : 0u;
   }
   F = bk::warp_sum(F); E = bk::warp_sum(E); oorf = bk::warp_sum(oorf);
   if ((threadIdx.x & 31) == 0) {
     if (F) atomicAdd(out, F);
-    if (E) atomicAdd(out + 1, (unsigned long long)E);
+    if (E) atomicAdd(out + 1, E);
     if (oorf) atomicOr(out + 2, 1ull);
   }
 }
diff --git a/breakid_b200/csrc/bkid_dist.cuh b/breakid_b200/csrc/bkid_dist.cuh
--- a/breakid_b200/csrc/bkid_dist.cuh
+++ b/breakid_b200/csrc/bkid_dist.cuh
@@ -362,7 +362,7 @@
   const double mean = (double)(long long)S / (double)(long long)N;
   const int kub = sd_upper_binade(S, N, SQ, gxm);
   const long long local_insert = c->cnt_insert;
-  TRY(c, sd_fast_launch(c, mean, kub, c->st2));
+  TRY(c, sd_hist_launch(c, mean, kub, c->st2));
   std::vector<uint64_t> ns(W);
   { uint64_t mine = (uint64_t)c->n; if (cm->allgather_host(&mine, 1, ns.data())) return fail(c, BKID_ERR_CUDA, "count exchange failed: " + cm->err); }
   unsigned long long offset = 0;
@@ -382,7 +382,7 @@
   TRY(c, exchange_rows(c, cm, c->dist_send, soff, (int)sizeof(bkid_cand), c->dist_recv, &nc_all));
   tm.a2a_cand = ms_since(t0); t0 = now();
   unsigned long long F = 0, E = 0;
-  TRY(c, sd_fast_collect(c, c->st2, &F, &E));
+  TRY(c, sd_hist_collect(c, c->st2, &F, &E));
   unsigned long long fe[2] = {F, E == ~0ull ? (1ull << 40) : std::min<unsigned long long>(E, 1ull << 40)};
   if (local_insert <= 0) { fe[0] = 0; fe[1] = 0; }
   CU(c, cudaMemcpyAsync(dv + 16, fe, 16, cudaMemcpyHostToDevice, st));
```
